# om-ai-lab/OmChat

Hardware: AMD Instinct MI355X
Metric: images/sec prefill + decode tokens/sec, OmChat-13B TP=1/8; p50 TTFT (higher is better)
Workload: dtype bf16

## Files before the change

### include/omchat_hip.h

```cpp
#ifndef OMCHAT_HIP_H
#define OMCHAT_HIP_H
#include <stddef.h>
#include <stdint.h>

#ifdef __cplusplus
extern "C" {
#endif

#define OMCHAT_F16 0
#define OMCHAT_BF16 1
#define OMCHAT_F32 2
#define OMCHAT_PAD_ROW INT32_MIN

typedef struct omchat_ctx omchat_ctx;

typedef struct {
  int v_hidden;
  int v_heads;
  int v_qk_channels;
  int v_mlp;
  int v_layers;
  int v_patch;
  int v_image;
  float v_eps;
// ... 53 lines not shown
                        const int32_t* seen_ids, const int32_t* n_seen_per_row, void* stream);
int omchat_set_sampling_filters(omchat_ctx* ctx, double min_p, double typical_p, double epsilon_cutoff, double eta_cutoff, void* stream);
int omchat_sample(omchat_ctx* ctx, const float* logits, int b, int32_t* next_tokens, void* stream);
#define OMCHAT_CON_MAX_NGRAM 64
#define OMCHAT_CON_MAX_EOS 16
#define OMCHAT_CON_MAX_SUPPRESS 1024
#define OMCHAT_CON_MAX_BAD_WORDS 1024
#define OMCHAT_CON_MAX_BAD_WORD_IDS 8192
int omchat_set_constraints(omchat_ctx* ctx, int b, int no_repeat_ngram_size, int min_new_tokens, int min_length, const int32_t* eos_ids, int n_eos,
                           const int32_t* suppress_ids, int n_suppress, const int32_t* begin_suppress_ids, int n_begin_suppress,
                           const int32_t* bad_word_ids, const int32_t* bad_word_offsets, int n_bad_words, const int32_t* prompt_ids,
                           const int32_t* prompt_len, int max_new, void* stream);
#define OMCHAT_FSM_MAX_STATES (1 << 20)
#define OMCHAT_FSM_MAX_EDGES (1 << 26)
#define OMCHAT_FSM_DEAD (-1)
int omchat_fsm_load(omchat_ctx* ctx, int n_states, const int32_t* off, const int32_t* tok, const int32_t* nxt, void* stream);
int omchat_fsm_begin(omchat_ctx* ctx, int b, const int32_t* start_states, int max_new, void* stream);
int omchat_fsm_states(omchat_ctx* ctx, int b, int32_t* out, void* stream);
int omchat_set_logprobs(omchat_ctx* ctx, int b, int max_new, void* stream);
int omchat_read_logprobs(omchat_ctx* ctx, int b, float* raw, float* processed, int32_t* counts, int max_len);
#define OMCHAT_LP_MAX_TOP 20
#define OMCHAT_LP_MAX_SCORED 32
int omchat_set_logprobs_ex(omchat_ctx* ctx, int b, int max_new, int top_n, const int32_t* score_ids, int n_score, void* stream);
int omchat_read_logprob_extras(omchat_ctx* ctx, int b, float* top_vals, int32_t* top_ids, float* scored, int32_t* counts, int max_len);
int omchat_read_sampling_state(omchat_ctx* ctx, int row, int* step, uint32_t* seen_words);
int omchat_kv_lengths(omchat_ctx* ctx, int32_t* out, int b);
int omchat_kv_rewind(omchat_ctx* ctx, int b, int n, void* stream);

int omchat_beam_begin(omchat_ctx* ctx, int b, int num_beams, float length_penalty, int early_stopping, const int32_t* eos_ids, int n_eos,
                      int max_new, int prompt_tok_len, void* stream);
int omchat_beam_step(omchat_ctx* ctx, const float* logits, int rows, int32_t* next_tokens, int32_t* done_word, void* stream);
int omchat_beam_result(omchat_ctx* ctx, int num_return, int32_t* tokens, int32_t* lengths, float* scores, int max_len);

int omchat_group_begin(omchat_ctx* ctx, int b, int N, int prompt_len, int share, void* stream);
int omchat_group_share_available(omchat_ctx* ctx, int N);

#define OMCHAT_VERIFY_KEEP_ALL 1
#define OMCHAT_VERIFY_SAMPLE 2
int omchat_decode_verify(omchat_ctx* ctx, const int32_t* tokens, int T, float* logits, int32_t* picks,
                         int* n_accept, int flags, void* stream);

int omchat_prefill_extend(omchat_ctx* ctx, const void* embeds, int S_new, int keep, float* logits_last, void* hidden_out, void* stream);
int omchat_extend_attn_form(int S_new, int keep, int Hkv);
int omchat_kv_read(omchat_ctx* ctx, int layer, int which, int pos0, int n, void* out, void* stream);
int omchat_kv_read_row(omchat_ctx* ctx, int row, int layer, int which, int pos0, int n, void* out, void* stream);

int omchat_prefill_suffixes(omchat_ctx* ctx, const void* embeds, int N, int S_max, const int32_t* lengths, int keep, float* logits_last,
                            void* hidden_out, void* stream);
int omchat_suffix_attn_form(int shared, int n_rep);

int omchat_enable_decode_graph(omchat_ctx* ctx, int on);
int omchat_decode_graph_stats(omchat_ctx* ctx, long* steps, long* replays, long* captures);
int omchat_bf16x12_stats(omchat_ctx* ctx, int* roles, long* launches, int* coded);

int omchat_enable_fp8_decode(omchat_ctx* ctx, int on);

int omchat_enable_mxfp4_decode(omchat_ctx* ctx, int mode);

enum omchat_weight_format {
  OMCHAT_WFMT_16 = 0,
  OMCHAT_WFMT_16_PACKED = 1,
  OMCHAT_WFMT_E4M3 = 2,
  OMCHAT_WFMT_MXFP4 = 3,
  OMCHAT_WFMT_MXFP4_PACKED = 4,
  OMCHAT_WFMT_COUNT = 5
};
int omchat_decode_weight_format(int rows, int fp8_on, int mxfp4_mode, int packed16_ready, int geometry_ok, int* x_pack_nb);

int omchat_enable_fp8_kv(omchat_ctx* ctx, int on);
int omchat_enable_fp8_prefill(omchat_ctx* ctx, int on);

#define OMCHAT_PROF_DECODE_GATEUP 0
#define OMCHAT_PROF_PREFILL_GATEUP 1
#define OMCHAT_PROF_VIT_FC1 2
#define OMCHAT_PROF_CATS 3
int omchat_prof_enable(omchat_ctx* ctx, int on);
int omchat_prof_read(omchat_ctx* ctx, int cat, double* total_ms, long* launches, int reset);

int omchat_mha_fwd(const void* qkv, int B, int S, int H, float softmax_scale, int causal, void* out, int dtype, void* stream);
int omchat_mha_fwd_varlen(const void* qkv, int B, int S, int H, int D, const int32_t* seqlens, float softmax_scale, int causal,
                          void* out, int dtype, void* stream);

int omchat_op_gemm(int dtype, const void* A, int lda, const void* W, int ldw, void* C, int ldc, int M, int N, int K,
                   const void* bias, const void* ls, const void* resid, int ldr, int epi, int force_tile, void* stream);
int omchat_op_gemm_fused(int dtype, const void* A, int lda, const void* W, int ldw, void* C, int ldc, int M, int N, int K,
                         const void* bias, const void* ls, const void* resid, int ldr, int epi, int force_tile, const float* row_scale,
                         const float* rs_stats, int rs_ld, int rs_nslots, int rs_dim, float rs_eps,
                         float* stats, int stats_ld, int* nslots, void* stream);
int omchat_op_stats_finish(const float* stats, int ld, int slot0, int nslots, int ngroups, int rows, int dim, float eps, float* out, void* stream);
int omchat_op_row_sumsq(int dtype, const void* x, int ldx, int rows, int H, float* stats, void* stream);
int omchat_op_fold_cols(int dtype, const void* W, const void* n, void* out, int rows, int cols, void* stream);
int omchat_op_vit_knorm_slots(int dtype, void* k, int ld, const void* wk, int rows, int C, int C_total, float eps, const float* stats, int stats_ld,
                              int nslots, float* sumsq_q, void* stream);
int omchat_op_mha_qnorm(int dtype, const void* qkv, int B, int Sq, int H, const float* sumsq, int stride, int dim, const void* wq,
                        float eps, float q_scale, void* out, void* stream);
int omchat_op_gemv_norm(int dtype, const void* X, const void* W, int ldw, void* Y, int N, int K, const void* norm_w, float eps,
                        const void* bias, int epi, int out_f32, void* stream);
int omchat_op_set_tuning(int key, int value);
int omchat_gemm_tune_load(const char* path);
int omchat_gemm_tune_dump(const char* path);
long omchat_gemm_tune_runs(void);
size_t omchat_op_gemm_sk_ws(void);
int omchat_op_gemm_sk(int dtype, const void* A, int lda, const void* W, int ldw, void* C, int ldc, int M, int N, int K,
                      const void* bias, const void* ls, const void* resid, int ldr, int epi, int force_tile, void* ws,
                      size_t ws_bytes, int stream_k, void* stream);
int omchat_op_gemv(int dtype, const void* X, int ldx, const void* W, int ldw, void* Y, int ldy, int b, int N, int K,
                   const void* bias, const void* resid, int ldr, int epi, int out_f32, void* stream);
int omchat_op_gemv_packed(int dtype, const void* X, int ldx, const void* W, int ldw, void* Y, int ldy, int b, int N, int K,
                          const void* bias, int epi, int out_f32, int ksplit, int w_packed, int y_packed, void* stream);
int omchat_op_pack_x(int dtype, const void* X, int ldx, int b, int K, void* out, void* stream);
int omchat_op_gemm_fp8(int dtype, const void* A8, const float* a_scale, const void* W8, const float* w_scale, void* C, int ldc, int M, int N,
                       int K, const void* bias, const void* resid, int ldr, int epi, void* stream);
int omchat_op_quant_rows_fp8(int dtype, const void* x, const void* norm_w, float eps, void* y8, float* scale, int rows, int H, void* stream);
int omchat_op_quant_fp8(int dtype, const void* W, int N, int K, void* W8, float* scale, void* stream);
int omchat_op_gemv_fp8(int dtype, const void* X, const void* W8, const float* scale, void* Y, int N, int K, const void* bias,
                       const void* resid, int epi, int out_f32, int ksplit, void* stream);
int omchat_op_quant_mxfp4(int dtype, const void* W, int N, int K, void* W4, void* S, void* stream);
int omchat_op_gemv_mxfp4(int dtype, const void* X, const void* W4, const void* S, void* Y, int N, int K, const void* bias,
                         const void* resid, int epi, int out_f32, int ksplit, void* stream);
int omchat_op_gemv_mxfp4_norm(int dtype, const void* X, const void* W4, const void* S, void* Y, int N, int K, const void* norm_w, float eps,
                              const void* bias, int epi, int out_f32, void* stream);
int omchat_op_gemv_mxfp4_rows(int dtype, const void* X, int ldx, const void* W4, const void* S, void* Y, int ldy, int b, int N, int K,
                              const void* bias, int epi, int out_f32, int ksplit, void* stream);
int omchat_op_gemv_mxfp4_packed(int dtype, const void* X, int ldx, const void* W4, const void* S, void* Y, int ldy, int b, int N, int K,
                                const void* bias, int epi, int out_f32, int ksplit, int y_packed, void* stream);
int omchat_op_encode_bf16x12(const void* W, int N, int K, void* coded, void* top, void* cnt, void* patch, void* over, void* stream);
int omchat_op_gemv_bf16x12(const void* X, const void* coded, const void* top, const void* cnt, const void* patch, void* Y, int N, int K,
                           const void* norm_w, float eps, const void* resid, int epi, int out_f32, void* stream);
int omchat_op_pack_w(int dtype, const void* W, int ldw, int N, int K, void* out, void* stream);
int omchat_op_pack_w4(const void* W4, const void* S, int N, int K, void* W4P, void* SP, void* stream);
int omchat_op_gemv_prepacked(int dtype, const void* XP, const void* WP, const void* SP, void* Y, int ldy, int b, int N, int K, const void* bias,
                             int epi, int out_f32, int ksplit, int y_packed, void* stream);
int omchat_op_rmsnorm(int dtype, const void* x, const void* w, void* y, int rows, int H, float eps, void* stream);
int omchat_op_resid_rmsnorm(int dtype, void* x, int ldx, const float* part, int ks, const void* w, void* xn, int ldn, int rows, int H,
                            float eps, int pack_nb, void* stream);
int omchat_op_vit_qknorm(int dtype, void* qkv, int ld, const void* wq, const void* wk, int rows, int C, int C_total,
                         float eps, float q_scale, void* stream);
int omchat_op_attn_prefill(int dtype, const void* q, const void* k, const void* v, void* out, int b, int Sq, int Skv,
                           int Hq, int Hkv, const int32_t* kv_len, int causal, int q_pos0, float scale, void* stream);
int omchat_op_attn_prefill_d(int dtype, const void* q, const void* k, const void* v, void* out, int b, int Sq, int Skv,
                             int Hq, int Hkv, int D, const int32_t* kv_len, int causal, int q_pos0, float scale, void* stream);
int omchat_op_layernorm(int dtype, const void* x, const void* w, const void* b, void* y, int rows, int H, float eps, void* stream);
size_t omchat_op_attn_decode_ws(int b, int Hq, int L);
int omchat_op_attn_decode(int dtype, const void* q, const void* k, const void* v, void* out, int b, int Hq, int Hkv,
                          int cap, int L, const int32_t* kv_len, float scale, void* ws, size_t ws_bytes, void* stream);
int omchat_op_attn_verify(int dtype, const void* q, void* k, void* v, void* out, int T, int Hq, int Hkv, int cap, int L, float scale,
                          void* ws, size_t ws_bytes, void* stream);
int omchat_op_attn_verify_tpw(int keys, int Hkv);
size_t omchat_op_attn_extend_ws(int Sq, int Hq, int Hkv, int L);
int omchat_op_attn_extend(int dtype, const void* q, const void* k, const void* v, void* out, int Sq, int Hq, int Hkv, int cap, int L,
                          float scale, void* ws, size_t ws_bytes, void* stream);
size_t omchat_op_attn_shared_ws(int G, int N, int Hq, int Hkv, int P, int L);
int omchat_op_attn_shared(int dtype, const void* q, void* k, void* v, void* out, int G, int N, int Hq, int Hkv, int cap, int P, int L,
                          float scale, void* ws, size_t ws_bytes, void* stream);
int omchat_op_attn_shared_lens(int dtype, const void* q, void* k, void* v, void* out, int G, int N, int Hq, int Hkv, int cap, int P, int L,
                               const int* kv_len, float scale, void* ws, size_t ws_bytes, void* stream);
size_t omchat_op_attn_suffix_ws(int N, int S, int Hq, int Hkv, int P);
int omchat_op_attn_suffix(int dtype, const void* q, const void* k, const void* v, void* out, int N, int S, int Hq, int Hkv, int cap, int P,
                          const int32_t* lengths, int* kv_len_dev, float scale, void* ws, size_t ws_bytes, void* stream);
int omchat_op_attn_verify_append(int dtype, const void* qkv, float theta, void* k, void* v, void* out, int T, int Hq, int Hkv, int cap,
                                 int L, float scale, void* ws, size_t ws_bytes, void* stream);
int omchat_op_attn_decode_kv8(int dtype, const void* q, const void* k8, const void* v8, const float* ks, const float* vs, void* out, int b,
                              int Hq, int Hkv, int cap, int L, const int32_t* kv_len, float scale, void* ws, size_t ws_bytes, void* stream);
int omchat_op_attn_decode_kv8_append(int dtype, void* qkv, float theta, void* k8, void* v8, float* ks, float* vs, void* k16, void* v16, void* out,
                                     int b, int Hq, int Hkv, int cap, int L, const int32_t* kv_len, const int32_t* pos, float scale, void* ws,
                                     size_t ws_bytes, void* stream);
int omchat_op_rope_kv(int dtype, void* qkv, int b, int S, int Hq, int Hkv, int pos0, float theta, void* kcache, void* vcache,
                      int cap, void* stream);
int omchat_op_rope_kv_q8(int dtype, void* qkv, int b, int S, int Hq, int Hkv, int pos0, float theta, void* kcache, void* vcache, int cap,
                         void* k8, void* v8, float* ks, float* vs, void* stream);
int omchat_op_argmax(const float* logits, int b, int V, int32_t* out, void* stream);
int omchat_op_attn_prefill_left(int dtype, const void* q, const void* k, const void* v, void* out, int b, int Sq, int Skv, int Hq, int Hkv,
                                const int32_t* kv_len, const int32_t* kv_start, int causal, int q_pos0, float scale, int fill_uniform, void* stream);
int omchat_op_rope_kv_pos(int dtype, void* qkv, int b, int S, int Hq, int Hkv, const int32_t* pos, int pos0, int slot0, int max_pos, float theta,
                          void* kcache, void* vcache, int cap, void* stream);
int omchat_op_argmax_ld(const float* logits, int ld, int b, int V, int32_t* out, int32_t* adv_pos, int32_t* adv_len, void* stream);
int omchat_op_im2col(int dtype, const void* pixels, void* cols, int B, int HW, int patch, int Kpad, void* stream);
int omchat_op_vit_assemble(int dtype, const void* pe, const void* cls, const void* pos, void* x, int B, int np, int C, void* stream);
int omchat_op_gather_rows(int dtype, const int32_t* idx, const void* table, const void* feats, void* out, int rows, int H, void* stream);
int omchat_op_copy_rows(int dtype, const void* src, int64_t src_ld, void* dst, int64_t dst_ld, int rows, int H, int group, int skip, void* stream);
int omchat_op_tp_finish(int dtype, const float* sum, const void* bias, const void* ls, const void* resid, void* out, int M, int N, int epi, void* stream);
// ... 82 lines not shown
```

### omchat_amd/_lib.py

```python
import ctypes as C
import os

HERE = os.path.dirname(os.path.abspath(__file__))
LIB_PATH = os.environ.get("OMCHAT_LIB") or os.path.join(HERE, "lib", "libomchat_hip.so")
_lib = None

F16, BF16, F32 = 0, 1, 2
EPI_NONE, EPI_GELU, EPI_LS_RESID, EPI_RESID, EPI_SWIGLU = 0, 1, 2, 3, 4
EPI_F32OUT = 6
EPI_LS_RESID_STATS, EPI_NONE_STATS = 7, 8
PAD_ROW = -(2 ** 31)
PROF_DECODE_GATEUP, PROF_PREFILL_GATEUP, PROF_VIT_FC1 = 0, 1, 2


class OmchatConfig(C.Structure):
    _fields_ = [
        ("v_hidden", C.c_int), ("v_heads", C.c_int), ("v_qk_channels", C.c_int), ("v_mlp", C.c_int), ("v_layers", C.c_int),
        ("v_patch", C.c_int), ("v_image", C.c_int), ("v_eps", C.c_float),
        ("t_hidden", C.c_int), ("t_layers", C.c_int), ("t_heads", C.c_int), ("t_kv_heads", C.c_int), ("t_mlp", C.c_int),
        ("t_vocab", C.c_int), ("t_vocab_total", C.c_int), ("t_eps", C.c_float), ("rope_theta", C.c_float),
        ("max_seq", C.c_int), ("max_batch", C.c_int), ("max_tiles", C.c_int), ("max_prefill_rows", C.c_int), ("dtype", C.c_int),
        ("v_head_dim", C.c_int), ("v_norm_type", C.c_int), ("v_no_qk_norm", C.c_int),
    ]

# ... 43 lines not shown
    "omchat_beam_step": (_i, [_vp, _vp, _i, _vp, _vp, _vp]),
    "omchat_beam_result": (_i, [_vp, _i, _vp, _vp, _vp, _i]),
    "omchat_decode_verify": (_i, [_vp, _vp, _i, _vp, _vp, _vp, _i, _vp]),
    "omchat_decode_step_masked": (_i, [_vp, _vp, _i, _vp, _vp, _i, _vp, _vp, _vp]),
    "omchat_masked_decode_begin": (_i, [_vp, _i, _vp, _vp, _i, _i, _vp]),
    "omchat_decode_step_masked_next": (_i, [_vp, _vp, _i, _vp, _vp, _vp]),
    "omchat_fused_status": (_i, [_vp, C.POINTER(C.c_long), C.POINTER(C.c_uint)]),
    "omchat_has_experiments": (_i, []),
    "omchat_set_allreduce_hook": (_i, [_vp, _vp, _vp]),
    "omchat_allreduce_noop": (_i, [_vp, _vp, C.c_size_t, _i, _vp]),
    "omchat_op_gemv_norm": (_i, [_i, _vp, _vp, _i, _vp, _i, _i, _vp, _f, _vp, _i, _i, _vp]),
    "omchat_prof_enable": (_i, [_vp, _i]),
    "omchat_prof_read": (_i, [_vp, _i, C.POINTER(C.c_double), C.POINTER(C.c_long), _i]),
    "omchat_mha_fwd": (_i, [_vp, _i, _i, _i, _f, _i, _vp, _i, _vp]),
    "omchat_mha_fwd_varlen": (_i, [_vp, _i, _i, _i, _i, _vp, _f, _i, _vp, _i, _vp]),
    "omchat_op_gemm": (_i, [_i, _vp, _i, _vp, _i, _vp, _i, _i, _i, _i, _vp, _vp, _vp, _i, _i, _i, _vp]),
    "omchat_op_gemm_fused": (_i, [_i, _vp, _i, _vp, _i, _vp, _i, _i, _i, _i, _vp, _vp, _vp, _i, _i, _i, _vp, _vp, _i, _i, _i, _f, _vp, _i, _vp, _vp]),
    "omchat_op_stats_finish": (_i, [_vp, _i, _i, _i, _i, _i, _i, _f, _vp, _vp]),
    "omchat_op_row_sumsq": (_i, [_i, _vp, _i, _i, _i, _vp, _vp]),
    "omchat_op_fold_cols": (_i, [_i, _vp, _vp, _vp, _i, _i, _vp]),
    "omchat_op_vit_knorm_slots": (_i, [_i, _vp, _i, _vp, _i, _i, _i, _f, _vp, _i, _i, _vp, _vp]),
    "omchat_op_mha_qnorm": (_i, [_i, _vp, _i, _i, _i, _vp, _i, _i, _vp, _f, _f, _vp, _vp]),
    "omchat_ctx_sp_stats": (_i, [_vp, C.POINTER(C.c_long), C.POINTER(C.c_long)]),
    "omchat_op_set_tuning": (_i, [_i, _i]),
    "omchat_gemm_tune_load": (_i, [C.c_char_p]),
    "omchat_gemm_tune_dump": (_i, [C.c_char_p]),
    "omchat_gemm_tune_runs": (C.c_long, []),
    "omchat_op_gemm_sk_ws": (_sz, []),
    "omchat_op_gemm_sk": (_i, [_i, _vp, _i, _vp, _i, _vp, _i, _i, _i, _i, _vp, _vp, _vp, _i, _i, _i, _vp, _sz, _i, _vp]),
    "omchat_op_gemv": (_i, [_i, _vp, _i, _vp, _i, _vp, _i, _i, _i, _i, _vp, _vp, _i, _i, _i, _vp]),
    "omchat_op_gemv_packed": (_i, [_i, _vp, _i, _vp, _i, _vp, _i, _i, _i, _i, _vp, _i, _i, _i, _i, _i, _vp]),
    "omchat_op_pack_x": (_i, [_i, _vp, _i, _i, _i, _vp, _vp]),
    "omchat_op_gemm_fp8": (_i, [_i, _vp, _vp, _vp, _vp, _vp, _i, _i, _i, _i, _vp, _vp, _i, _i, _vp]),
    "omchat_op_quant_rows_fp8": (_i, [_i, _vp, _vp, _f, _vp, _vp, _i, _i, _vp]),
    "omchat_enable_fp8_decode": (_i, [_vp, _i]),
    "omchat_enable_fp8_kv": (_i, [_vp, _i]),
    "omchat_enable_fp8_prefill": (_i, [_vp, _i]),
    "omchat_enable_decode_graph": (_i, [_vp, _i]),
    "omchat_bf16x12_stats": (_i, [_vp, C.POINTER(_i), C.POINTER(C.c_long), C.POINTER(_i)]),
    "omchat_decode_graph_stats": (_i, [_vp, C.POINTER(C.c_long), C.POINTER(C.c_long), C.POINTER(C.c_long)]),
    "omchat_op_quant_fp8": (_i, [_i, _vp, _i, _i, _vp, _vp, _vp]),
    "omchat_op_gemv_fp8": (_i, [_i, _vp, _vp, _vp, _vp, _i, _i, _vp, _vp, _i, _i, _i, _vp]),
    "omchat_enable_mxfp4_decode": (_i, [_vp, _i]),
    "omchat_decode_weight_format": (_i, [_i, _i, _i, _i, _i, C.POINTER(_i)]),
    "omchat_op_quant_mxfp4": (_i, [_i, _vp, _i, _i, _vp, _vp, _vp]),
    "omchat_op_gemv_mxfp4": (_i, [_i, _vp, _vp, _vp, _vp, _i, _i, _vp, _vp, _i, _i, _i, _vp]),
    "omchat_op_gemv_mxfp4_rows": (_i, [_i, _vp, _i, _vp, _vp, _vp, _i, _i, _i, _i, _vp, _i, _i, _i, _vp]),
    "omchat_op_gemv_mxfp4_packed": (_i, [_i, _vp, _i, _vp, _vp, _vp, _i, _i, _i, _i, _vp, _i, _i, _i, _i, _vp]),
    "omchat_op_pack_w": (_i, [_i, _vp, _i, _i, _i, _vp, _vp]),
    "omchat_op_pack_w4": (_i, [_vp, _vp, _i, _i, _vp, _vp, _vp]),
    "omchat_op_gemv_prepacked": (_i, [_i, _vp, _vp, _vp, _vp, _i, _i, _i, _i, _vp, _i, _i, _i, _i, _vp]),
    "omchat_op_encode_bf16x12": (_i, [_vp, _i, _i, _vp, _vp, _vp, _vp, _vp, _vp]),
    "omchat_op_gemv_bf16x12": (_i, [_vp, _vp, _vp, _vp, _vp, _vp, _i, _i, _vp, _f, _vp, _i, _i, _vp]),
    "omchat_op_gemv_mxfp4_norm": (_i, [_i, _vp, _vp, _vp, _vp, _i, _i, _vp, _f, _vp, _i, _i, _vp]),
    "omchat_op_rmsnorm": (_i, [_i, _vp, _vp, _vp, _i, _i, _f, _vp]),
    "omchat_op_resid_rmsnorm": (_i, [_i, _vp, _i, _vp, _i, _vp, _vp, _i, _i, _i, _f, _i, _vp]),
    "omchat_op_vit_qknorm": (_i, [_i, _vp, _i, _vp, _vp, _i, _i, _i, _f, _f, _vp]),
    "omchat_op_attn_prefill": (_i, [_i, _vp, _vp, _vp, _vp, _i, _i, _i, _i, _i, _vp, _i, _i, _f, _vp]),
    "omchat_op_attn_prefill_d": (_i, [_i, _vp, _vp, _vp, _vp, _i, _i, _i, _i, _i, _i, _vp, _i, _i, _f, _vp]),
    "omchat_op_layernorm": (_i, [_i, _vp, _vp, _vp, _vp, _i, _i, _f, _vp]),
    "omchat_op_attn_decode_ws": (_sz, [_i, _i, _i]),
    "omchat_op_attn_decode": (_i, [_i, _vp, _vp, _vp, _vp, _i, _i, _i, _i, _i, _vp, _f, _vp, _sz, _vp]),
    "omchat_op_attn_verify_tpw": (_i, [_i, _i]),
    "omchat_op_attn_verify": (_i, [_i, _vp, _vp, _vp, _vp, _i, _i, _i, _i, _i, _f, _vp, _sz, _vp]),
    "omchat_op_attn_extend_ws": (_sz, [_i, _i, _i, _i]),
    "omchat_op_attn_shared_ws": (_sz, [_i, _i, _i, _i, _i, _i]),
    "omchat_op_attn_shared": (_i, [_i, _vp, _vp, _vp, _vp, _i, _i, _i, _i, _i, _i, _i, _f, _vp, _sz, _vp]),
    "omchat_op_attn_extend": (_i, [_i, _vp, _vp, _vp, _vp, _i, _i, _i, _i, _i, _f, _vp, _sz, _vp]),
    "omchat_prefill_extend": (_i, [_vp, _vp, _i, _i, _vp, _vp, _vp]),
    "omchat_extend_attn_form": (_i, [_i, _i, _i]),
    "omchat_kv_read": (_i, [_vp, _i, _i, _i, _i, _vp, _vp]),
    "omchat_kv_read_row": (_i, [_vp, _i, _i, _i, _i, _i, _vp, _vp]),
    "omchat_prefill_suffixes": (_i, [_vp, _vp, _i, _i, _vp, _i, _vp, _vp, _vp]),
    "omchat_suffix_attn_form": (_i, [_i, _i]),
    "omchat_op_attn_shared_lens": (_i, [_i, _vp, _vp, _vp, _vp, _i, _i, _i, _i, _i, _i, _i, _vp, _f, _vp, _sz, _vp]),
    "omchat_op_attn_suffix_ws": (_sz, [_i, _i, _i, _i, _i]),
    "omchat_op_attn_suffix": (_i, [_i, _vp, _vp, _vp, _vp, _i, _i, _i, _i, _i, _i, _vp, _vp, _f, _vp, _sz, _vp]),
    "omchat_op_attn_verify_append": (_i, [_i, _vp, _f, _vp, _vp, _vp, _i, _i, _i, _i, _i, _f, _vp, _sz, _vp]),
    "omchat_op_attn_decode_kv8": (_i, [_i, _vp, _vp, _vp, _vp, _vp, _vp, _i, _i, _i, _i, _i, _vp, _f, _vp, _sz, _vp]),
    "omchat_op_attn_decode_kv8_append": (_i, [_i, _vp, _f, _vp, _vp, _vp, _vp, _vp, _vp, _vp, _i, _i, _i, _i, _i, _vp, _vp, _f, _vp, _sz, _vp]),
    "omchat_op_rope_kv": (_i, [_i, _vp, _i, _i, _i, _i, _i, _f, _vp, _vp, _i, _vp]),
    "omchat_op_rope_kv_q8": (_i, [_i, _vp, _i, _i, _i, _i, _i, _f, _vp, _vp, _i, _vp, _vp, _vp, _vp, _vp]),
    "omchat_op_argmax": (_i, [_vp, _i, _i, _vp, _vp]),
    "omchat_op_attn_prefill_left": (_i, [_i, _vp, _vp, _vp, _vp, _i, _i, _i, _i, _i, _vp, _vp, _i, _i, _f, _i, _vp]),
    "omchat_op_rope_kv_pos": (_i, [_i, _vp, _i, _i, _i, _i, _vp, _i, _i, _i, _f, _vp, _vp, _i, _vp]),
    "omchat_op_argmax_ld": (_i, [_vp, _i, _i, _i, _vp, _vp, _vp, _vp]),
    "omchat_op_im2col": (_i, [_i, _vp, _vp, _i, _i, _i, _i, _vp]),
    "omchat_op_vit_assemble": (_i, [_i, _vp, _vp, _vp, _vp, _i, _i, _i, _vp]),
    "omchat_op_gather_rows": (_i, [_i, _vp, _vp, _vp, _vp, _i, _i, _vp]),
    "omchat_op_copy_rows": (_i, [_i, _vp, _i64, _vp, _i64, _i, _i, _i, _i, _vp]),
    "omchat_op_tp_finish": (_i, [_i, _vp, _vp, _vp, _vp, _vp, _i, _i, _i, _vp]),
    "omchat_op_resid16_norm": (_i, [_i, _vp, _i, _vp, _i, _vp, _vp, _vp, _i, _i, _i, _f, _vp]),
    "omchat_op_cast_f32": (_i, [_i, _vp, _vp, _i64, _vp]),
    "omchat_op_rmsnorm_ld": (_i, [_i, _vp, _i, _vp, _vp, _i, _i, _i, _f, _i, _vp]),
    "omchat_op_layernorm_ld": (_i, [_i, _vp, _i, _vp, _vp, _vp, _i, _i, _i, _f, _vp]),
    "omchat_op_sample": (_i, [_vp, _i, _i, _u64, _f, _i, C.c_double, _f, _vp, _vp, _i, _vp, _vp, _vp]),
    "omchat_op_token_logprob": (_i, [_vp, _i, _i, _i, _vp, _vp, _f, _f, _vp, _vp, _vp, _vp, _vp, _vp, _vp]),
    "omchat_op_lse_label_ws": (_sz, [_i, _i]),
    "omchat_op_lse_label": (_i, [_i, _vp, _i, _vp, _i, _i, _i, _i, _vp, _vp, _vp, _vp, _sz, _vp]),
    "omchat_op_top_logprobs": (_i, [_vp, _i, _i, _i, _i, _vp, _i, _vp, _vp, _vp, _vp]),
    "omchat_op_sample_filtered": (_i, [_vp, _i, _i, _u64, _f, _i, C.c_double, _f, C.c_double, C.c_double, C.c_double, C.c_double, _vp, _vp, _i,
                                       _vp, _vp, _vp, _vp]),
    "omchat_op_sample_verify": (_i, [_vp, _i, _i, _i, _vp, _u64, _i, _f, _i, C.c_double, _f, C.c_double, C.c_double, C.c_double, C.c_double, _vp,
                                     _i, _i, _i, _vp, _vp, _vp, _vp]),
    "omchat_read_sampling_state": (_i, [_vp, _i, _vp, _vp]),
    "omchat_op_token_logprob_interval": (_i, [_vp, _i, _i, _i, _vp, _vp, _f, _f, _vp, _vp, _vp, _vp, _vp, _vp, _vp, _vp]),
# ... 83 lines not shown
```

### omchat_amd/csrc/capi.hip

```cpp
#include "kernels.h"
#include <stdlib.h>
#include "../../include/omchat_hip.h"
#include <math.h>
#include <vector>

#define S(x) ((hipStream_t)(x))
#if OMCHAT_EXPERIMENTS
int g_launch_any_order = 0;
#endif

extern "C" int omchat_op_gemm(int dtype, const void* A, int lda, const void* W, int ldw, void* C, int ldc, int M, int N, int K,
                              const void* bias, const void* ls, const void* resid, int ldr, int epi, int force_tile, void* stream) {
  GemmArgs g{A, lda, W, ldw, C, ldc, M, N, K, bias, ls, resid, ldr, epi, force_tile, nullptr, 0, -1};
  return launch_gemm(dtype, g, S(stream));
}

extern "C" int omchat_op_gemm_fused(int dtype, const void* A, int lda, const void* W, int ldw, void* C, int ldc, int M, int N, int K,
                                    const void* bias, const void* ls, const void* resid, int ldr, int epi, int force_tile, const float* row_scale,
                                    const float* rs_stats, int rs_ld, int rs_nslots, int rs_dim, float rs_eps,
                                    float* stats, int stats_ld, int* nslots, void* stream) {
  GemmArgs g{A, lda, W, ldw, C, ldc, M, N, K, bias, ls, resid, ldr, epi, force_tile, nullptr, 0, -1};
  g.row_scale = row_scale; g.stats = stats; g.stats_ld = stats_ld; g.stats_nslots = nslots;
  g.rs_stats = rs_stats; g.rs_ld = rs_ld; g.rs_nslots = rs_nslots; g.rs_dim = rs_dim; g.rs_eps = rs_eps;
  return launch_gemm(dtype, g, S(stream));
// ... 20 lines not shown
  a.K = (const char*)qkv + (size_t)H * 128 * 2; a.k_sb = a.q_sb; a.k_sh = 128; a.k_sr = row;
  a.V = (const char*)qkv + (size_t)2 * H * 128 * 2; a.v_sb = a.q_sb; a.v_sh = 128; a.v_sr = row;
  a.O = out; a.o_sb = (int64_t)Sq * H * 128; a.o_sh = 128; a.o_sr = (int64_t)H * 128;
  a.batch = B; a.q_heads = H; a.kv_heads = H; a.Sq = Sq; a.Skv = Sq; a.kv_len = nullptr; a.causal = 0; a.q_pos0 = 0;
  a.scale = 1.0f;
  a.qn_sumsq = sumsq; a.qn_stride = stride; a.qn_dim = dim; a.qn_w = wq; a.qn_eps = eps; a.qn_scale = q_scale;
  return launch_attn_prefill(dtype, a, S(stream));
}

extern "C" int omchat_op_set_tuning(int key, int value) {
  const char* allow = getenv("OMCHAT_ALLOW_TUNING");
  if (!allow || allow[0] != '1') {
    omchat_set_error("omchat_op_set_tuning: process-global test / measurement hook; set OMCHAT_ALLOW_TUNING=1 to use it (see include/omchat_hip.h)");
    return 1;
  }
  if (key == 0) { gemm_set_skew(value); return 0; }
  if (key == 1) { gemv_set_force_mfma(value); return 0; }
  if (key == 5) { gemm_set_autotune(value); return 0; }
  if (key == 4) { model_set_ar_min_rows(value); return 0; }
  if (key == 6) { model_set_pack_replica(value); return 0; }
  if (key == 8) { attn_set_v2(value); return 0; }
  if (key == 9) { model_set_fuse_peer_norm(value); return 0; }
  if (key == 10) { attn_set_tpw(value); return 0; }
  if (key == 11) { gemv_set_no_xs(value); return 0; }
  if (key == 12) { attn_set_klds(value); return 0; }
  if (key == 25) { attn_set_dma(value); return 0; }
  if (key == 26) { attn_set_dma_slots(value); return 0; }
  if (key == 27) { attn_set_dma_rot(value); return 0; }
  if (key == 28) { gemv_set_skew(value); return 0; }
  if (key == 29) { model_set_tp_f32(value); return 0; }
  if (key == 30) { attn_set_hsplit(value); return 0; }
  if (key == 33) { attn_set_mha_xcd(value); return 0; }
  if (key == 16) { gemv_set_norm_loop(value); return 0; }
  if (key == 17) { gemv_set_rows_balance(value); return 0; }
  if (key == 19) { attn_set_merge_mid_min(value); return 0; }
  if (key == 21) { attn_set_merge_dg(value); return 0; }
  if (key == 13) { gemm_set_persist(value); return 0; }
  if (key == 14) { model_set_norm_in_gemv(value); return 0; }
  if (key == 22) { model_set_fuse_attn_oproj(value); return 0; }
  if (key == 23) { model_set_decode_layer(value); return 0; }
  if (key == 24) { gemv_set_dyn(value); return 0; }
  if (key == 34) { gemv_set_shard_shapes(value); return 0; }
  if (key == 35) { model_set_shard_as_tp1(value); return 0; }
  if (key == 36) { attn_set_kg(value); return 0; }
  if (key == 37) { gemm_set_wide_store(value); return 0; }
  if (key == 43) { gemm_set_skip_dead(value); return 0; }
  if (key == 44) { model_set_vit_fused(value); return 0; }
  if (key == 45) { model_set_tp_sp(value); return 0; }
  if (key == 46) { attn_set_peel(value); return 0; }
  if (key == 47) { attn_set_kv8_tpw(value); return 0; }
  if (key == 48) { attn_set_kv8_fuse(value); return 0; }
  if (key == 49) { model_set_extend_attn(value); return 0; }
  if (key == 50) { model_set_x12_roles(value); return 0; }
  if (key == 51) { model_set_suffix_attn(value); return 0; }
  if (key == 38) { gemv_set_gu_rr(value); return 0; }
  if (key == 39) { gemv_set_longk_direct(value); return 0; }
  if (key == 40) { norm_set_wave(value); return 0; }
#if OMCHAT_EXPERIMENTS
  if (key == 41) { g_launch_any_order = value; return 0; }
  if (key == 42) { model_set_ao_oproj(value); return 0; }
#endif
  omchat_set_error("omchat_op_set_tuning: unknown key");
  return 1;
}

extern "C" int omchat_allreduce_noop(void*, void*, size_t, int, void*) { return 0; }

extern "C" int omchat_gemm_tune_load(const char* path) { OM_CHECK(path, "null path"); return gemm_tune_load(path); }
extern "C" int omchat_gemm_tune_dump(const char* path) { OM_CHECK(path, "null path"); return gemm_tune_dump(path); }
extern "C" long omchat_gemm_tune_runs(void) { return gemm_tune_runs(); }

extern "C" size_t omchat_op_gemm_sk_ws(void) { return gemm_sk_ws_bytes(); }

extern "C" int omchat_op_gemm_sk(int dtype, const void* A, int lda, const void* W, int ldw, void* C, int ldc, int M, int N, int K,
                                 const void* bias, const void* ls, const void* resid, int ldr, int epi, int force_tile, void* ws,
                                 size_t ws_bytes, int stream_k, void* stream) {
  GemmArgs g{A, lda, W, ldw, C, ldc, M, N, K, bias, ls, resid, ldr, epi, force_tile, ws, ws_bytes, stream_k};
  return launch_gemm(dtype, g, S(stream));
}

extern "C" int omchat_op_gemv(int dtype, const void* X, int ldx, const void* W, int ldw, void* Y, int ldy, int b, int N, int K,
                              const void* bias, const void* resid, int ldr, int epi, int out_f32, void* stream) {
  GemvArgs g{X, ldx, W, ldw, Y, ldy, b, N, K, bias, resid, ldr, epi, out_f32};
  return launch_gemv(dtype, g, S(stream));
}

extern "C" int omchat_op_gemv_norm(int dtype, const void* X, const void* W, int ldw, void* Y, int N, int K, const void* norm_w, float eps,
                                   const void* bias, int epi, int out_f32, void* stream) {
  OM_CHECK(X && W && Y && norm_w, "null argument");
  GemvArgs g{X, K, W, ldw, Y, N, 1, N, K, bias, nullptr, 0, epi, out_f32};
  g.norm_w = norm_w; g.norm_eps = eps;
  return launch_gemv(dtype, g, S(stream));
}

extern "C" int omchat_op_gemv_packed(int dtype, const void* X, int ldx, const void* W, int ldw, void* Y, int ldy, int b, int N, int K,
                                     const void* bias, int epi, int out_f32, int ksplit, int w_packed, int y_packed, void* stream) {
  OM_CHECK(b >= 1 && b <= 32 && K % 64 == 0, "1 <= b <= 32, K % 64 == 0");
  const int NB = b > 16 ? 2 : 1;
  void *xp = nullptr, *wp = nullptr;
  OM_HIP(hipMalloc(&xp, (size_t)NB * 16 * K * 2));
  int rc = launch_pack_x(dtype, X, ldx, b, K, xp, S(stream));
  if (rc == 0 && w_packed) {
    if (hipMalloc(&wp, (size_t)N * K * 2) != hipSuccess) { hipFree(xp); omchat_set_error("hipMalloc failed"); return 2; }
    rc = launch_pack_w(dtype, W, ldw, N, K, wp, S(stream));
  }
  if (rc == 0) {
// ... 698 lines not shown
  const int NB = b > 16 ? 2 : 1;
  void *xp = nullptr, *wp = nullptr, *sp = nullptr;
  auto drop = [&]() { if (xp) hipFree(xp); if (wp) hipFree(wp); if (sp) hipFree(sp); };
  if (hipMalloc(&xp, (size_t)NB * 16 * K * 2) != hipSuccess || hipMalloc(&wp, (size_t)N * (K / 2)) != hipSuccess ||
      hipMalloc(&sp, (size_t)N * (K / 32)) != hipSuccess) {
    (void)hipGetLastError(); drop(); omchat_set_error("hipMalloc failed"); return 2;
  }
  int rc = launch_pack_x(dtype, X, ldx, b, K, xp, S(stream));
  if (rc == 0) rc = launch_pack_w4(W4, (const unsigned char*)S_, N, K, wp, (unsigned char*)sp, S(stream));
  if (rc == 0) {
    GemvArgs g{xp, K, wp, K / 2, Y, ldy, b, N, K, bias, nullptr, 0, epi, out_f32, ksplit, 0, nullptr, 1, 1, y_packed};
    g.mx_scale = (const unsigned char*)sp;
    rc = launch_gemv(dtype, g, S(stream));
  }
  hipStreamSynchronize(S(stream));
  drop();
  return rc;
}

extern "C" int omchat_op_pack_w(int dtype, const void* W, int ldw, int N, int K, void* out, void* stream) { return launch_pack_w(dtype, W, ldw, N, K, out, S(stream)); }
extern "C" int omchat_op_pack_w4(const void* W4, const void* S_, int N, int K, void* W4P, void* SP, void* stream) {
  return launch_pack_w4(W4, (const unsigned char*)S_, N, K, W4P, (unsigned char*)SP, S(stream));
}
extern "C" int omchat_op_gemv_prepacked(int dtype, const void* XP, const void* WP, const void* SP, void* Y, int ldy, int b, int N, int K, const void* bias,
                                        int epi, int out_f32, int ksplit, int y_packed, void* stream) {
  OM_CHECK(XP && WP && Y, "null argument");
  OM_CHECK(b >= 1 && b <= 32 && K >= 64 && K % 64 == 0 && N >= 16 && N % 16 == 0, "pre-packed GEMV: 1 <= b <= 32, K % 64 == 0, N % 16 == 0");
  GemvArgs g{XP, K, WP, SP ? K / 2 : K, Y, ldy, b, N, K, bias, nullptr, 0, epi, out_f32, ksplit, 0, nullptr, 1, 1, y_packed};
  g.mx_scale = (const unsigned char*)SP;
  return launch_gemv(dtype, g, S(stream));
}

extern "C" int omchat_op_gemv_mxfp4_norm(int dtype, const void* X, const void* W4, const void* S_, void* Y, int N, int K, const void* norm_w,
                                         float eps, const void* bias, int epi, int out_f32, void* stream) {
  OM_CHECK(X && W4 && S_ && Y && norm_w, "null argument");
  OM_CHECK(K % 32 == 0, "MXFP4: K must be a multiple of 32 (one e8m0 scale per 32 consecutive k)");
  GemvArgs g{X, K, W4, K / 2, Y, N, 1, N, K, bias, nullptr, 0, epi, out_f32};
  g.norm_w = norm_w; g.norm_eps = eps;
  g.mx_scale = (const unsigned char*)S_;
  return launch_gemv(dtype, g, S(stream));
}

extern "C" int omchat_op_encode_bf16x12(const void* W, int N, int K, void* coded, void* top, void* cnt, void* patch, void* over, void* stream) {
  return launch_encode_bf16x12(W, K, N, K, coded, (unsigned char*)top, (unsigned char*)cnt, (unsigned*)patch, (int*)over, S(stream));
}
extern "C" int omchat_op_gemv_bf16x12(const void* X, const void* coded, const void* top, const void* cnt, const void* patch, void* Y, int N, int K,
                                      const void* norm_w, float eps, const void* resid, int epi, int out_f32, void* stream) {
  OM_CHECK(X && coded && top && cnt && patch && Y, "null argument");
  GemvArgs g{X, K, coded, K / 2 * 3, Y, N, 1, N, K, nullptr, resid, N, epi, out_f32};
  g.norm_w = norm_w; g.norm_eps = eps;
  g.x12_top = (const unsigned char*)top; g.x12_cnt = (const unsigned char*)cnt; g.x12_patch = (const unsigned*)patch;
  return launch_gemv(OMCHAT_BF16, g, S(stream));
}

extern "C" int omchat_op_attn_prefill_d(int dtype, const void* q, const void* k, const void* v, void* out, int b, int Sq, int Skv, int Hq,
                                        int Hkv, int D, const int32_t* kv_len, int causal, int q_pos0, float scale, void* stream) {
  AttnArgs a{};
  a.Q = q; a.q_sb = (int64_t)Sq * Hq * D; a.q_sh = D; a.q_sr = (int64_t)Hq * D;
  a.K = k; a.k_sb = (int64_t)Hkv * Skv * D; a.k_sh = (int64_t)Skv * D; a.k_sr = D;
  a.V = v; a.v_sb = a.k_sb; a.v_sh = a.k_sh; a.v_sr = D;
  a.O = out; a.o_sb = a.q_sb; a.o_sh = D; a.o_sr = a.q_sr;
  a.batch = b; a.q_heads = Hq; a.kv_heads = Hkv; a.Sq = Sq; a.Skv = Skv; a.kv_len = kv_len; a.causal = causal; a.q_pos0 = q_pos0; a.scale = scale;
  a.head_dim = D;
  return launch_attn_prefill(dtype, a, S(stream));
}

extern "C" int omchat_op_layernorm(int dtype, const void* x, const void* w, const void* b, void* y, int rows, int H, float eps, void* stream) {
  return launch_layernorm(dtype, x, H, w, b, y, H, rows, H, eps, S(stream));
}

extern "C" int omchat_op_attn_prefill_left(int dtype, const void* q, const void* k, const void* v, void* out, int b, int Sq, int Skv, int Hq,
                                           int Hkv, const int32_t* kv_len, const int32_t* kv_start, int causal, int q_pos0, float scale,
                                           int fill_uniform, void* stream) {
  OM_CHECK(q && k && v && out && kv_start, "null argument");
  AttnArgs a{};
  a.Q = q; a.q_sb = (int64_t)Sq * Hq * 128; a.q_sh = 128; a.q_sr = (int64_t)Hq * 128;
  a.K = k; a.k_sb = (int64_t)Hkv * Skv * 128; a.k_sh = (int64_t)Skv * 128; a.k_sr = 128;
  a.V = v; a.v_sb = a.k_sb; a.v_sh = a.k_sh; a.v_sr = 128;
  a.O = out; a.o_sb = a.q_sb; a.o_sh = 128; a.o_sr = a.q_sr;
  a.batch = b; a.q_heads = Hq; a.kv_heads = Hkv; a.Sq = Sq; a.Skv = Skv; a.kv_len = kv_len; a.kv_start = kv_start; a.causal = causal;
  a.q_pos0 = q_pos0; a.scale = scale;
  int rc = launch_attn_prefill(dtype, a, S(stream));
  if (!rc && fill_uniform) rc = launch_attn_uniform_rows(dtype, a, S(stream));
  return rc;
}

extern "C" int omchat_op_rope_kv_pos(int dtype, void* qkv, int b, int Sq, int Hq, int Hkv, const int32_t* pos, int pos0, int slot0, int max_pos,
                                     float theta, void* kcache, void* vcache, int cap, void* stream) {
  OM_CHECK(qkv && kcache && vcache && b >= 1 && Sq >= 1 && Hq >= 1 && Hkv >= 1 && max_pos >= 1 && cap >= 1 && slot0 >= -1, "bad argument");
  if (pos) {
    std::vector<int32_t> hp((size_t)b * Sq);
    OM_HIP(hipStreamSynchronize(S(stream)));
    OM_HIP(hipMemcpy(hp.data(), pos, hp.size() * 4, hipMemcpyDeviceToHost));
    for (int32_t p : hp) {
      OM_CHECK(p >= 0 && p < max_pos, "position outside the RoPE table");
      OM_CHECK(slot0 >= 0 || p < cap, "cache slot exceeds the capacity");
    }
  } else {
    OM_CHECK(pos0 >= 0 && pos0 + Sq <= max_pos, "position outside the RoPE table");
    OM_CHECK(slot0 >= 0 || pos0 + Sq <= cap, "cache slot exceeds the capacity");
  }
  OM_CHECK(slot0 < 0 || slot0 + Sq <= cap, "cache slot exceeds the capacity");
  float* d = rope_table_device(max_pos, theta);
  OM_CHECK(d, "rope table allocation failed");
  RopeArgs r{qkv, (Hq + 2 * Hkv) * 128, b * Sq, Sq, Hq, Hkv, pos, pos0, d, max_pos, kcache, vcache, (int64_t)Hkv * cap * 128, (int64_t)cap * 128};
  r.slot0 = slot0;
// ... 57 lines not shown
```

### omchat_amd/csrc/ctx.h

```cpp
#pragma once
#include "kernels.h"
#include "../../include/omchat_hip.h"
#include <rccl/rccl.h>
#include <string>
#include <unordered_map>
#include <vector>

#define TRY(x) do { int rc_ = (x); if (rc_) return rc_; } while (0)

extern int g_fuse_peer_norm;

enum RouteKind { R_PLAIN = 0, R_GATE = 1, R_UP = 2, R_PATCH = 3 };
struct Route {
  void* dst = nullptr;
  int64_t rows = 0, cols = 0;
  int64_t dst_ld = 0;
  int kind = R_PLAIN;
  bool loaded = false;
  float synth_std = 0.02f, synth_off = 0.f;
};

struct Grown {
  void* p = nullptr; size_t cap = 0;
  void release() { if (p) (void)hipFree(p); p = nullptr; cap = 0; }
// ... 54 lines not shown
  int fsm_cap = 0, fsm_fed = 0;
  int *fsm_cnt = nullptr;
  int32_t* fsm_cur = nullptr;
  uint32_t* fsm_bm = nullptr; int fsm_bmw = 0;
  bool sampling_on() const { return smp.on; }
  bool constraints_on() const { return con.on; }
  bool logprobs_on() const { return lp.on; }
  bool fsm_on() const { return fsm.on; }
  void release() { con_hist.release(); lp_rec.release(); lp_xrec.release(); fsm_mem.release(); fsm_trail.release(); }
};

struct BeamState {
  struct Search { bool on = false; int b = 0, N = 0, KB = 0, max_new = 0, P = 0, es = 0, ns = 1, t = 0; float lp = 1.f; std::vector<int> eos; };
  Search cur;
  Grown state, table, dn, parents, stash;
  bool stash8 = false;
  std::vector<int> hpos, hlen;
  bool on() const { return cur.on; }
  void end() { cur.on = false; }
  void release() { for (Grown* g : {&state, &table, &dn, &parents, &stash}) g->release(); }
};

struct GroupState {
  bool share = false; int b = 0, N = 0, P = 0;
  Grown ws;
  std::vector<int> hpos, hlen;
  bool on() const { return share; }
  void end() { share = false; }
  void release() { ws.release(); }
};

struct omchat_ctx {
  omchat_config c;
  int dt = OMCHAT_BF16;
  int tp_rank = 0, tp_size = 1;
  ncclComm_t comm = nullptr;
  std::vector<void*> allocs;
  size_t bytes = 0;
  std::unordered_map<std::string, Route> routes;

  int v_np = 0, v_ntok = 0, v_Cq = 0, v_kpad = 0, v_hd = 128;
  int t_qdim = 0, t_kvdim = 0, t_qkvdim = 0;

  struct VitLayer { void *ls1, *ls2, *n1, *n2, *n1b, *n2b, *wqkv, *qn, *kn, *wproj, *bproj, *w1, *b1, *w2, *b2; };
  struct DecLayer { void *ln1, *ln2, *wqkv, *bqkv, *wo, *wgu, *wd; };
  enum Proj { P_QKV = 0, P_O = 1, P_GU = 2, P_DOWN = 3, P_LM = 4 };
  struct WRef { void* W = nullptr; int ldw = 0; float* w_scale = nullptr; unsigned char* mx_scale = nullptr; int packed = 0; };
  enum WState { W_ABSENT = 0, W_BUILT, W_STALE, W_UNAVAILABLE };
  struct WTable { std::vector<WRef> e; int state = W_ABSENT; };
  WTable wt[OMCHAT_WFMT_COUNT];
  const WRef* layer_w(int fmt, int layer) const { return &wt[fmt].e[(size_t)layer * 4]; }
  const WRef& lm_w(int fmt) const { return wt[fmt].e.back(); }
  bool built(int fmt) const { return wt[fmt].state == W_BUILT; }
  enum X12Role { X12_GU = 0, X12_DOWN = 1, X12_LM = 2, X12_ROLES = 3 };
  struct X12Ref { void* W = nullptr; unsigned char* top = nullptr; unsigned char* cnt = nullptr; unsigned* patch = nullptr; bool ok = false; };
  struct X12Table { std::vector<X12Ref> e; int state = W_ABSENT; };
  X12Table x12[X12_ROLES];
  int* x12_over = nullptr;
  long x12_launches[X12_ROLES] = {0, 0, 0};
  bool fp8_decode = false;
  int mxfp4_mode = 0;
  void *k8cache = nullptr, *v8cache = nullptr;
  float *ks8 = nullptr, *vs8 = nullptr;
  bool fp8_kv = false, kv8_valid = false, fp8_prefill = false;
  void* tw_q8 = nullptr; float* tw_q8s = nullptr;
  int64_t scale_layer_stride() const { return (int64_t)c.max_batch * c.t_kv_heads * c.max_seq; }
  struct DecodeGraph { hipGraph_t graph = nullptr; hipGraphExec_t exec = nullptr; int cap_len = 0, grp_N = 0, grp_P = 0; const void* grp_ws = nullptr; };
  std::unordered_map<int, DecodeGraph> graphs;
  bool graph_on = false;
  hipStream_t graph_stream = nullptr;
  hipEvent_t graph_ev_in = nullptr, graph_ev_out = nullptr;
  int32_t *d_tok_in = nullptr, *d_tok_out = nullptr;
  long graph_steps = 0, graph_replays = 0, graph_captures = 0;
  void *v_cls = nullptr, *v_pos = nullptr, *v_wpatch = nullptr, *v_bpatch = nullptr;
  std::vector<VitLayer> vl;
  void *p_w0 = nullptr, *p_b0 = nullptr, *p_w2 = nullptr, *p_b2 = nullptr;
  void *t_embed = nullptr, *t_norm = nullptr, *t_lm = nullptr;
  std::vector<DecLayer> dl;
  float* rope = nullptr;

  void *vw_cols = nullptr, *vw_pe = nullptr, *vw_x = nullptr, *vw_x2 = nullptr, *vw_xn = nullptr, *vw_qkv = nullptr, *vw_ao = nullptr,
       *vw_h = nullptr, *vw_feat = nullptr, *vw_proj = nullptr;
  float* vw_sumsq = nullptr;
  float *vw_stats_x = nullptr, *vw_stats_qk = nullptr, *vw_rstd = nullptr;
  int vw_stats_x_ld = 0, vw_stats_qk_ld = 0, vw_stats_x_ld_used = 1;
  struct VitFold { void *wqkv = nullptr, *w1 = nullptr; };
  std::vector<VitFold> vfold;
  bool vfold_stale = true;
  void *tw_x = nullptr, *tw_x2 = nullptr, *tw_xn = nullptr, *tw_qkv = nullptr, *tw_ao = nullptr, *tw_act = nullptr, *tw_last = nullptr;
  float* tw_logits = nullptr;
  void* sk_ws = nullptr; size_t sk_ws_bytes = 0;
  float* tp_f32_ws = nullptr; size_t tp_f32_bytes = 0;
  float* tw_part = nullptr;
  float* tw_attn_ws = nullptr;
  size_t tw_attn_ws_bytes = 0;
  void* fd_ws = nullptr;
  unsigned* fd_err = nullptr;
  unsigned fd_epoch = 0;
  long n_fused_launches = 0;
  void* dl_ws = nullptr;
  long n_layer_launches = 0;
  unsigned long long* dbg_stamps = nullptr;
  unsigned* dyn_ctr = nullptr;
  int *d_pos = nullptr, *d_len = nullptr, *d_idx = nullptr, *d_start = nullptr;
  int* d_verify_n = nullptr;
  PickState pick;
  BeamState beam;
  GroupState group;
  Grown ext_ws;
  Grown score_ws;
  int grow(Grown& g, size_t n) {
    if (n <= g.cap) return 0;
// ... 168 lines not shown
```

### omchat_amd/csrc/gemv.hip

```cpp
#include "kernels.h"
#include "rowdot.h"
#include <type_traits>

namespace {

struct GemvP {
  const void* X; const void* W; void* Y; const void* bias; const void* resid;
  int ldx, ldw, ldy, ldr, b, N, K, out_f32, ksplit;
  const float* w_scale;
  int y_packed;
  const void* norm_w; float norm_eps;
  unsigned* dyn;
  void* y_pack;
  unsigned long long* dbg;
  const unsigned char* mx_s;
  const unsigned char* x12_top;
  const unsigned char* x12_cnt;
  const unsigned* x12_patch;
#if OMCHAT_EXPERIMENTS
  int xskew;
#endif
};
constexpr int WF_16 = 0, WF_E4M3 = 1, WF_MX4 = 2, WF_X12 = 3;
#if OMCHAT_EXPERIMENTS
// ... 653 lines not shown
  s.pv = p.x12_patch[row * 32 + (lane & 31)];
}
__device__ __forceinline__ void x12_row_finish(X12Row& s) {
  const int t = __builtin_amdgcn_readfirstlane((int)s.top_raw) - 7;
  s.cnt = __builtin_amdgcn_readfirstlane((int)s.cnt_raw);
  s.pi = 0;
  s.tlo = ((unsigned)((t + 1) & 0x7f) << 8) | ((unsigned)((t + 2) & 0x7f) << 16) | ((unsigned)((t + 3) & 0x7f) << 24);
  s.thi = (unsigned)((t + 4) & 0x7f) | ((unsigned)((t + 5) & 0x7f) << 8) | ((unsigned)((t + 6) & 0x7f) << 16) | ((unsigned)((t + 7) & 0x7f) << 24);
}
__device__ __forceinline__ rw_u32x4 x12_decode(const X12W& w, const X12Row& s) {
  const unsigned n = w.nib;
  const unsigned c0 = n & 0x07070707u, c1 = (n >> 4) & 0x07070707u;
  unsigned h0 = __builtin_amdgcn_perm(s.thi, s.tlo, c0), h1 = __builtin_amdgcn_perm(s.thi, s.tlo, c1);
  h0 |= (n & 0x08080808u) << 4;
  h1 |= n & 0x80808080u;
  rw_u32x4 r;
  r.x = __builtin_amdgcn_perm(h0, w.lo.x, 0x05010400u);
  r.y = __builtin_amdgcn_perm(h0, w.lo.x, 0x07030602u);
  r.z = __builtin_amdgcn_perm(h1, w.lo.y, 0x05010400u);
  r.w = __builtin_amdgcn_perm(h1, w.lo.y, 0x07030602u);
  return r;
}
__device__ __forceinline__ void x12_apply(rw_u32x4& w, unsigned e, int lane) {
  const unsigned k = e >> 16, i = k & 7u, sh = (i & 1u) * 16u;
  const unsigned keep = ~(0xffffu << sh), ins = (e & 0xffffu) << sh;
  const bool mine = lane == (int)((k >> 3) & 63u);
  w.x = (mine && (i >> 1) == 0u) ? ((w.x & keep) | ins) : w.x;
  w.y = (mine && (i >> 1) == 1u) ? ((w.y & keep) | ins) : w.y;
  w.z = (mine && (i >> 1) == 2u) ? ((w.z & keep) | ins) : w.z;
  w.w = (mine && (i >> 1) == 3u) ? ((w.w & keep) | ins) : w.w;
}
template <int G>
__device__ __forceinline__ void x12_group(rw_u32x4 (&wd)[G], const X12W* w, X12Row& s, int chunk0, int nch, int lane) {
#pragma unroll
  for (int i = 0; i < G; ++i) wd[i] = x12_decode(w[i], s);
  while (s.pi < s.cnt) {
    const unsigned e = (unsigned)__builtin_amdgcn_readlane((int)s.pv, s.pi);
    const int ch = (int)(e >> 25) - chunk0;
    if (ch >= G) break;
#pragma unroll
    for (int i = 0; i < G; ++i) if (ch == i) x12_apply(wd[i], e, lane);
    ++s.pi;
  }
  if (chunk0 + G > nch) {
    for (int j = 0; j < s.cnt; ++j) {
      const unsigned e = (unsigned)__builtin_amdgcn_readlane((int)s.pv, j);
      if ((e >> 19) != 0u) break;
#pragma unroll
      for (int i = 0; i < G; ++i) if (chunk0 + i >= nch) x12_apply(wd[i], e, 0);
    }
  }
}

template <typename T, int WF>
__device__ __forceinline__ typename RwW<WF>::type rw_ldw(const GemvP& p, size_t row, int k) {
  if constexpr (WF == WF_X12) return x12_ldw(p, row, k >> 9, (k >> 3) & 63); else
  if constexpr (WF == WF_E4M3) {
    return __builtin_nontemporal_load(reinterpret_cast<const rw_u32x2*>((const unsigned char*)p.W + row * p.ldw + k));
  } else if constexpr (WF == WF_MX4) {
    rw_u32x2 w;
    w.x = __builtin_nontemporal_load(reinterpret_cast<const unsigned*>((const unsigned char*)p.W + row * p.ldw + (k >> 1)));
    w.y = __builtin_nontemporal_load(p.mx_s + row * (size_t)(p.K >> 5) + (k >> 5));
    return w;
  } else {
    return __builtin_nontemporal_load(reinterpret_cast<const rw_u32x4*>((const T*)p.W + row * p.ldw + k));
  }
}
template <typename T, int WF>
__device__ __forceinline__ float rw_dotw(typename RwW<WF>::type w, rw_u32x4 x, float acc) {
  if constexpr (WF == WF_E4M3) return rw_dot8_fp8<T>(w, x, acc);
  else if constexpr (WF == WF_MX4) return fmaf(rw_dot8_fp4<T>(w.x, x), mx_scale_of(w.y), acc);
  else return rw_dot8<T>(w, x, acc);
}

template <typename T, int R> struct RwTail { const T* p0; const T* p1; int idx[R]; float v0[R], v1[R]; };
template <typename T, int R> __device__ __forceinline__ void rw_tail_load(RwTail<T, R>& t) {
#pragma unroll
  for (int r = 0; r < R; ++r) { t.v0[r] = tof(t.p0[t.idx[r]]); t.v1[r] = tof(t.p1[t.idx[r]]); }
}
template <typename T, int R, int NCH, int WF>
__device__ __forceinline__ void rw_rows_q(const GemvP& p, const int (&rows)[R], int k0, int lane, const rw_u32x4 (&xr)[RW_MAXC], float (&acc)[R],
                                          RwTail<T, R>& tail) {
  typename RwW<WF>::type w[R][NCH];
#pragma unroll
  for (int r = 0; r < R; ++r)
#pragma unroll
    for (int c = 0; c < NCH; ++c) {
      int k = k0 + c * 512 + lane * 8;
      k = k < p.K ? k : k0;
      w[r][c] = rw_ldw<T, WF>(p, (size_t)rows[r], k);
    }
  float sc[R];
#pragma unroll
  for (int r = 0; r < R; ++r) sc[r] = WF == WF_E4M3 ? p.w_scale[rows[r]] : 1.f;
  rw_tail_load<T, R>(tail);
#pragma unroll
  for (int r = 0; r < R; ++r) {
    float a = 0.f;
#pragma unroll
    for (int c = 0; c < NCH; ++c) a = rw_dotw<T, WF>(w[r][c], xr[c], a);
#pragma unroll
    for (int o = 32; o > 0; o >>= 1) a += __shfl_xor(a, o, 64);
    acc[r] = WF == WF_E4M3 ? a * sc[r] : a;
  }
}

template <typename T, int R, int N, int WF>
__device__ __forceinline__ void rw_dispatch_q(int nch, const GemvP& p, const int (&rows)[R], int k0, int lane, const rw_u32x4 (&xr)[RW_MAXC],
                                              float (&acc)[R], RwTail<T, R>& tail) {
  if constexpr (N > 0) {
    if (nch == N) rw_rows_q<T, R, N, WF>(p, rows, k0, lane, xr, acc, tail);
    else rw_dispatch_q<T, R, N - 1, WF>(nch, p, rows, k0, lane, xr, acc, tail);
  }
}

template <typename T, int R, int NCH>
__device__ __forceinline__ void rw_rows(const T* W, int ldw, const int (&rows)[R], int k0, int K, int lane, const rw_u32x4 (&xr)[RW_MAXC],
                                        float (&acc)[R], RwTail<T, R>& tail) {
  rw_u32x4 w[R][NCH];
#pragma unroll
  for (int r = 0; r < R; ++r)
#pragma unroll
    for (int c = 0; c < NCH; ++c) {
      int k = k0 + c * 512 + lane * 8;
      k = k < K ? k : k0;
      w[r][c] = __builtin_nontemporal_load(reinterpret_cast<const rw_u32x4*>(W + (size_t)rows[r] * ldw + k));
    }
  rw_tail_load<T, R>(tail);
#pragma unroll
  for (int r = 0; r < R; ++r) {
    float a = 0.f;
#pragma unroll
    for (int c = 0; c < NCH; ++c) a = rw_dot8<T>(w[r][c], xr[c], a);
#pragma unroll
    for (int o = 32; o > 0; o >>= 1) a += __shfl_xor(a, o, 64);
    acc[r] = a;
  }
}

template <typename T, int R, int N>
__device__ __forceinline__ void rw_dispatch(int nch, const T* W, int ldw, const int (&rows)[R], int k0, int K, int lane,
                                            const rw_u32x4 (&xr)[RW_MAXC], float (&acc)[R], RwTail<T, R>& tail) {
  if constexpr (N > 0) {
    if (nch == N) rw_rows<T, R, N>(W, ldw, rows, k0, K, lane, xr, acc, tail);
    else rw_dispatch<T, R, N - 1>(nch, W, ldw, rows, k0, K, lane, xr, acc, tail);
  }
}

template <typename T, int EPI, int RR, int WAVES, int F8>
__device__ __forceinline__ void gemv_rows_body(const GemvP& p) {
  constexpr int R = EPI == EPI_SWIGLU ? 2 * RR : RR;
  constexpr int OUT = RR;
  const int lane = threadIdx.x & 63, wave = threadIdx.x >> 6;
  const T* W = (const T*)p.W;
  if constexpr (EPI == EPI_RESID && WAVES == 7) OM_DBG_MIN(1, blockIdx.x < 8);
  const int nch_all = (p.K + 511) / 512;
  const int c_lo = (int)(((long)nch_all * blockIdx.y) / p.ksplit), c_hi = (int)(((long)nch_all * (blockIdx.y + 1)) / p.ksplit);
  const int nch = c_hi - c_lo, k0 = c_lo * 512;
  rw_u32x4 xr[RW_MAXC];
#pragma unroll
  for (int c = 0; c < RW_MAXC; ++c) {
    const int k = k0 + c * 512 + lane * 8;
    rw_u32x4 z = {0u, 0u, 0u, 0u};
    xr[c] = (c < nch && k < p.K) ? *reinterpret_cast<const rw_u32x4*>((const T*)p.X + k) : z;
  }
  const int n_out = EPI == EPI_SWIGLU ? p.N / 2 : p.N;
  const int ngroups = (n_out + OUT - 1) / OUT;
  for (int g = blockIdx.x * WAVES + wave; g < ngroups; g += gridDim.x * WAVES) {
    int rows[R];
#pragma unroll
    for (int r = 0; r < R; ++r) {
      if constexpr (EPI == EPI_SWIGLU) {
        int n = g * RR + (r % RR); n = n < n_out ? n : n_out - 1;
        rows[r] = 32 * (n >> 4) + (n & 15) + (r / RR) * 16;
      } else {
        const int n = g * R + r;
        rows[r] = n < p.N ? n : p.N - 1;
      }
    }
    float acc[R];
    RwTail<T, R> tail;
    {
      constexpr bool plain = EPI != EPI_SWIGLU && EPI != EPI_PARTIAL;
      const bool hb = plain && p.bias, hr = EPI == EPI_RESID && !p.out_f32;
      tail.p0 = hb ? (const T*)p.bias : (const T*)p.X;
      tail.p1 = hr ? (const T*)p.resid : (const T*)p.X;
#pragma unroll
      for (int r = 0; r < R; ++r) {
        const int n = g * OUT + r;
        tail.idx[r] = (hb || hr) ? (n < n_out ? n : n_out - 1) : 0;
      }
      if (!hb) tail.p0 = tail.p1;
      if (!hr) tail.p1 = tail.p0;
    }
    if constexpr (F8 != WF_16) rw_dispatch_q<T, R, RW_MAXC, F8>(nch, p, rows, k0, lane, xr, acc, tail);
    else rw_dispatch<T, R, RW_MAXC>(nch, W, p.ldw, rows, k0, p.K, lane, xr, acc, tail);
    if (lane == 0) {
#pragma unroll
      for (int r = 0; r < OUT; ++r) {
        const int n = g * OUT + r;
        if (n >= n_out) continue;
        if constexpr (EPI == EPI_SWIGLU) {
          const float gt = rnd<T>(acc[r]), up = rnd<T>(acc[r + RR]);
          ((T*)p.Y)[n] = fromf<T>(rnd<T>(silu(gt)) * up);
        } else if constexpr (EPI == EPI_PARTIAL) {
          ((float*)p.Y)[(size_t)blockIdx.y * p.ldy + n] = acc[r];
        } else {
          float y = acc[r] + (p.bias ? tail.v0[r] : 0.f);
          if (p.out_f32) ((float*)p.Y)[n] = y;
          else {
            y = rnd<T>(y);
            if constexpr (EPI == EPI_RESID) y = tail.v1[r] + y;
            ((T*)p.Y)[n] = fromf<T>(y);
          }
        }
      }
    }
  }
  if constexpr (EPI == EPI_RESID && WAVES == 7) OM_DBG_MAX(3, (blockIdx.x & 7) == 0);
}

template <typename T, int EPI, int RR = 4, int WAVES = 4, bool F8 = false>
__global__ __launch_bounds__(WAVES * 64) void gemv_rows_kernel(GemvP p) { gemv_rows_body<T, EPI, RR, WAVES, F8 ? WF_E4M3 : WF_16>(p); }
template <typename T, int EPI, int RR, int WAVES>
__global__ __launch_bounds__(WAVES * 64) void gemv_rows_mx4_kernel(GemvP p) { gemv_rows_body<T, EPI, RR, WAVES, WF_MX4>(p); }

template <typename T, int EPI, int RR, int NCH, int F8, int WAVES>
__device__ __forceinline__ void gemv_rows_norm_body(const GemvP& p) {
  typedef typename V8<T>::type v8;
  constexpr int R = EPI == EPI_SWIGLU ? 2 * RR : RR;
  __shared__ __attribute__((aligned(16))) T xs[NCH * 512];
  __shared__ float red[WAVES];
  const int lane = threadIdx.x & 63, wave = __builtin_amdgcn_readfirstlane(threadIdx.x >> 6);
  const int n_out = EPI == EPI_SWIGLU ? p.N / 2 : p.N;
  int g = blockIdx.x * WAVES + wave;
#if OMCHAT_EXPERIMENTS
  if constexpr (EPI == EPI_SWIGLU && RR == 1 && WAVES == 4) {
    if (p.xskew) {
      const int x = blockIdx.x & 7, j = blockIdx.x >> 3;
      const int base = ((n_out + 3) / 4) / 8;
      const int n_x = base + ((x & 1) ? -p.xskew : p.xskew);
      if (j >= n_x) return;
      g = (x * base + ((x & 1) ? p.xskew : 0) + j) * 4 + wave;
    }
  }
#endif
  if constexpr (EPI == EPI_SWIGLU) OM_DBG_MIN(4, blockIdx.x < 8);
  if constexpr (EPI == EPI_NONE) OM_DBG_MIN(8, blockIdx.x < 8);
  static_assert(WAVES >= 4 && NCH <= 8, "sum-of-squares order: four owner waves, up to two chunks each");
  constexpr int MC = (NCH + WAVES - 1) / WAVES;
  constexpr int SC = (NCH + 3) / 4;
  rw_u32x4 xq[MC], nq[MC], sq[SC];
#pragma unroll
  for (int i = 0; i < MC; ++i) {
    const int c = wave + WAVES * i, k = c * 512 + lane * 8;
    const rw_u32x4 z = {0u, 0u, 0u, 0u};
    const bool ok = c < NCH && k < p.K;
    xq[i] = ok ? *reinterpret_cast<const rw_u32x4*>((const T*)p.X + k) : z;
    nq[i] = ok ? *reinterpret_cast<const rw_u32x4*>((const T*)p.norm_w + k) : z;
  }
#pragma unroll
  for (int i = 0; i < SC; ++i) {
    if constexpr (WAVES == 4) {
      sq[i] = xq[i];
    } else {
      const int c = wave + 4 * i, k = c * 512 + lane * 8;
      const rw_u32x4 z = {0u, 0u, 0u, 0u};
      sq[i] = (wave < 4 && c < NCH && k < p.K) ? *reinterpret_cast<const rw_u32x4*>((const T*)p.X + k) : z;
    }
  }
  int rows[R];
#pragma unroll
  for (int r = 0; r < R; ++r) {
    if constexpr (EPI == EPI_SWIGLU) {
      int n = g * RR + (r % RR); n = n < n_out ? n : n_out - 1;
      rows[r] = 32 * (n >> 4) + (n & 15) + (r / RR) * 16;
    } else {
      const int n = g * R + r;
      rows[r] = n < p.N ? n : p.N - 1;
    }
  }
  typedef typename RwW<F8>::type wreg_t;
  wreg_t w[R][NCH];
#pragma unroll
  for (int r = 0; r < R; ++r)
#pragma unroll
    for (int c = 0; c < NCH; ++c) {
      int k = c * 512 + lane * 8;
      k = k < p.K ? k : 0;
      if constexpr (F8 == WF_X12) w[r][c] = x12_ldw(p, (size_t)rows[r], c, lane);
      else w[r][c] = rw_ldw<T, F8>(p, (size_t)rows[r], k);
    }
  float e_bias[RR], e_scale[R];
  {
    const T* bp = (EPI != EPI_SWIGLU && p.bias) ? (const T*)p.bias : (const T*)p.norm_w;
    const int nmax = (EPI != EPI_SWIGLU && p.bias) ? n_out - 1 : 0;
#pragma unroll
    for (int r = 0; r < RR; ++r) {
      const int n = g * RR + r;
      e_bias[r] = tof(bp[n < nmax ? n : nmax]);
    }
    if (!(EPI != EPI_SWIGLU && p.bias)) {
#pragma unroll
      for (int r = 0; r < RR; ++r) e_bias[r] = 0.f;
    }
#pragma unroll
    for (int r = 0; r < R; ++r) e_scale[r] = 1.f;
    if constexpr (F8 == WF_E4M3) {
#pragma unroll
      for (int r = 0; r < R; ++r) e_scale[r] = p.w_scale[rows[r]];
    }
  }
  X12Row xst[F8 == WF_X12 ? R : 1];
  if constexpr (F8 == WF_X12) {
#pragma unroll
    for (int r = 0; r < R; ++r) x12_row_load(xst[r], p, (size_t)rows[r], lane);
  }
  __builtin_amdgcn_sched_barrier(0);
  float ss = 0.f;
#pragma unroll
  for (int i = 0; i < SC; ++i) {
    const v8 xv = __builtin_bit_cast(v8, sq[i]);
#pragma unroll
    for (int j = 0; j < 8; ++j) { const float v = tof(xv[j]); ss += v * v; }
  }
#pragma unroll
  for (int o = 32; o > 0; o >>= 1) ss += __shfl_xor(ss, o, 64);
  if (lane == 0 && wave < 4) red[wave] = ss;
  asm volatile("s_waitcnt lgkmcnt(0)" ::: "memory");
  __builtin_amdgcn_s_barrier();
  float tot = red[0];
#pragma unroll
  for (int w = 1; w < 4; ++w) tot += red[w];
  const float inv = rsqrtf(tot / (float)p.K + p.norm_eps);
#pragma unroll
  for (int i = 0; i < MC; ++i) {
    const int c = wave + WAVES * i;
    if (c < NCH) {
      const v8 xv = __builtin_bit_cast(v8, xq[i]), wv = __builtin_bit_cast(v8, nq[i]);
      v8 o;
#pragma unroll
      for (int j = 0; j < 8; ++j) o[j] = fromf<T>(tof(wv[j]) * rnd<T>(tof(xv[j]) * inv));
      *reinterpret_cast<v8*>(xs + c * 512 + lane * 8) = o;
    }
  }
  asm volatile("s_waitcnt lgkmcnt(0)" ::: "memory");
  __builtin_amdgcn_s_barrier();
  rw_u32x4 xr[NCH];
#pragma unroll
  for (int c = 0; c < NCH; ++c) xr[c] = *reinterpret_cast<const rw_u32x4*>(xs + c * 512 + lane * 8);
  __builtin_amdgcn_sched_barrier(0);
  float acc[R];
#pragma unroll
  for (int r = 0; r < R; ++r) {
    float a = 0.f;
    if constexpr (F8 == WF_X12) x12_row_finish(xst[r]);
#pragma unroll
    for (int c = 0; c < NCH; ++c) {
      if constexpr (F8 != WF_X12) a = rw_dotw<T, F8>(w[r][c], xr[c], a);
    }
    if constexpr (F8 == WF_X12) {
      constexpr int G0 = NCH < 4 ? NCH : 4, G1 = NCH - G0;
      {
        rw_u32x4 wd[G0];
        x12_group<G0>(wd, &w[r][0], xst[r], 0, NCH, lane);
#pragma unroll
        for (int c = 0; c < G0; ++c) a = rw_dot8<T>(wd[c], xr[c], a);
      }
      if constexpr (G1 > 0) {
        rw_u32x4 wd[G1];
        x12_group<G1>(wd, &w[r][G0], xst[r], G0, NCH, lane);
#pragma unroll
        for (int c = 0; c < G1; ++c) a = rw_dot8<T>(wd[c], xr[G0 + c], a);
      }
    }
#pragma unroll
    for (int o = 32; o > 0; o >>= 1) a += __shfl_xor(a, o, 64);
    if constexpr (F8 == WF_E4M3) a *= e_scale[r];
    acc[r] = a;
  }
  if (lane == 0) {
#pragma unroll
    for (int r = 0; r < RR; ++r) {
      const int n = g * RR + r;
      if (n >= n_out) continue;
      if constexpr (EPI == EPI_SWIGLU) {
        const float gt = rnd<T>(acc[r]), up = rnd<T>(acc[r + RR]);
        ((T*)p.Y)[n] = fromf<T>(rnd<T>(silu(gt)) * up);
      } else {
        const float y = acc[r] + e_bias[r];
        if (p.out_f32) ((float*)p.Y)[n] = y;
        else ((T*)p.Y)[n] = fromf<T>(y);
      }
    }
  }
  if constexpr (EPI == EPI_SWIGLU) { OM_DBG_MAX(5, blockIdx.x + 64 >= gridDim.x); OM_DBG_MAX(16 + (blockIdx.x & 7), blockIdx.x + 512 >= gridDim.x); }
  if constexpr (EPI == EPI_NONE) OM_DBG_MAX(9, (blockIdx.x & 7) == 0);
}

template <typename T, int EPI, int RR, int NCH, bool F8, int WAVES = 4>
__global__ __launch_bounds__(WAVES * 64) void gemv_rows_norm_kernel(GemvP p) { gemv_rows_norm_body<T, EPI, RR, NCH, F8 ? WF_E4M3 : WF_16, WAVES>(p); }
template <typename T, int EPI, int RR, int NCH, int WAVES = 4>
__global__ __launch_bounds__(WAVES * 64) void gemv_rows_norm_mx4_kernel(GemvP p) { gemv_rows_norm_body<T, EPI, RR, NCH, WF_MX4, WAVES>(p); }
template <typename T, int EPI, int RR, int NCH>
__global__ __launch_bounds__(256) void gemv_rows_norm_x12_kernel(GemvP p) { gemv_rows_norm_body<T, EPI, RR, NCH, WF_X12, 4>(p); }

template <typename T, int EPI, int NCH, int F8>
__device__ __forceinline__ void gemv_rows_norm_loop_body(const GemvP& p, int per_wg, unsigned skew) {
  typedef typename V8<T>::type v8;
  constexpr int R = EPI == EPI_SWIGLU ? 2 : 1;
  __shared__ __attribute__((aligned(16))) T xs[NCH * 512];
  __shared__ float red[4];
  const int lane = threadIdx.x & 63, wave = __builtin_amdgcn_readfirstlane(threadIdx.x >> 6);
  const int n_out = EPI == EPI_SWIGLU ? p.N / 2 : p.N;
  int o0 = blockIdx.x * per_wg, o1 = o0 + per_wg < n_out ? o0 + per_wg : n_out;
  if constexpr (EPI == EPI_SWIGLU) OM_DBG_MIN(4, blockIdx.x < 8);
  if (skew) {
    const int l = blockIdx.x & 7;
    int pre = 0;
    for (int i = 0; i < l; ++i) pre += per_wg + (int)((skew >> (4 * i)) & 15u) - 8;
    o0 = (blockIdx.x >> 3) * 8 * per_wg + pre;
    o1 = o0 + per_wg + (int)((skew >> (4 * l)) & 15u) - 8;
    o1 = o1 < n_out ? o1 : n_out;
  }
  typedef typename RwW<F8>::type wreg_t;
  auto row_of = [&](int n, int r) { return EPI == EPI_SWIGLU ? 32 * (n >> 4) + (n & 15) + r * 16 : n; };
  auto load_w = [&](wreg_t (&w)[R][NCH], int n) {
#pragma unroll
    for (int r = 0; r < R; ++r) {
      const size_t row = (size_t)row_of(n, r);
#pragma unroll
      for (int c = 0; c < NCH; ++c) {
        int k = c * 512 + lane * 8;
        k = k < p.K ? k : 0;
        w[r][c] = rw_ldw<T, F8>(p, row, k);
      }
    }
  };
  wreg_t wa[R][NCH], wb[R][NCH], wc[R][NCH];
  const int u0 = o0 + wave;
  if (u0 < o1) load_w(wa, u0);
  if (u0 + 4 < o1) load_w(wb, u0 + 4);
  if (u0 + 8 < o1) load_w(wc, u0 + 8);
  constexpr int MC = (NCH + 3) / 4;
  rw_u32x4 xq[MC], nq[MC];
#pragma unroll
  for (int i = 0; i < MC; ++i) {
    const int c = wave + 4 * i, k = c * 512 + lane * 8;
    const rw_u32x4 z = {0u, 0u, 0u, 0u};
    const bool ok = c < NCH && k < p.K;
    xq[i] = ok ? *reinterpret_cast<const rw_u32x4*>((const T*)p.X + k) : z;
    nq[i] = ok ? *reinterpret_cast<const rw_u32x4*>((const T*)p.norm_w + k) : z;
  }
  __builtin_amdgcn_sched_barrier(0);
  float ss = 0.f;
#pragma unroll
  for (int i = 0; i < MC; ++i) {
    const v8 xv = __builtin_bit_cast(v8, xq[i]);
// ... 462 lines not shown
      if constexpr (F8 == WF_MX4) hipLaunchKernelGGL((gemv_rows_norm_mx4_kernel<T, EPI, 1, NCH, 9>), dim3(2 * n_cu), dim3(576), 0, s, p);
      else hipLaunchKernelGGL((gemv_rows_norm_kernel<T, EPI, 1, NCH, F8 == WF_E4M3, 9>), dim3(2 * n_cu), dim3(576), 0, s, p);
      return;
    }
  }
#if OMCHAT_EXPERIMENTS
  if constexpr (EPI == EPI_SWIGLU && RR == 1) {
    const int nwg = cdiv(n_out, 4), xs = (int)(g_gemv_skew < 256u ? g_gemv_skew : 0u);
    if (xs > 0 && nwg % 8 == 0 && n_out % 4 == 0 && xs < nwg / 8) {
      GemvP q = p; q.xskew = xs;
      if constexpr (F8 == WF_MX4) hipLaunchKernelGGL((gemv_rows_norm_mx4_kernel<T, EPI, RR, NCH>), dim3(8 * (nwg / 8 + xs)), dim3(256), 0, s, q);
      else hipLaunchKernelGGL((gemv_rows_norm_kernel<T, EPI, RR, NCH, F8 == WF_E4M3>), dim3(8 * (nwg / 8 + xs)), dim3(256), 0, s, q);
      return;
    }
  }
#endif
  if constexpr (F8 == WF_MX4) hipLaunchKernelGGL((gemv_rows_norm_mx4_kernel<T, EPI, RR, NCH>), dim3(cdiv(cdiv(n_out, RR), 4)), dim3(256), 0, s, p);
  else hipLaunchKernelGGL((gemv_rows_norm_kernel<T, EPI, RR, NCH, F8 == WF_E4M3>), dim3(cdiv(cdiv(n_out, RR), 4)), dim3(256), 0, s, p);
}
template <typename T, int EPI, int RR, int F8>
void launch_rows_norm(const GemvP& p, hipStream_t s) {
  switch (cdiv(p.K, 512)) {
    case 1: launch_rows_norm_n<T, EPI, RR, F8, 1>(p, s); break;
    case 2: launch_rows_norm_n<T, EPI, RR, F8, 2>(p, s); break;
    case 3: launch_rows_norm_n<T, EPI, RR, F8, 3>(p, s); break;
    case 4: launch_rows_norm_n<T, EPI, RR, F8, 4>(p, s); break;
    case 5: launch_rows_norm_n<T, EPI, RR, F8, 5>(p, s); break;
    case 6: launch_rows_norm_n<T, EPI, RR, F8, 6>(p, s); break;
    case 7: launch_rows_norm_n<T, EPI, RR, F8, 7>(p, s); break;
    default: launch_rows_norm_n<T, EPI, RR, F8, 8>(p, s); break;
  }
}

template <int EPI, int NCH>
void launch_rows_norm_x12_n(const GemvP& p, hipStream_t s) {
  constexpr int RR = EPI == EPI_SWIGLU ? 1 : 4;
  const int n_out = EPI == EPI_SWIGLU ? p.N / 2 : p.N;
  hipLaunchKernelGGL((gemv_rows_norm_x12_kernel<bf16, EPI, RR, NCH>), dim3(cdiv(cdiv(n_out, RR), 4)), dim3(256), 0, s, p);
}
template <int EPI>
void launch_rows_norm_x12(const GemvP& p, hipStream_t s) {
  switch (p.K / 512) {
    case 1: launch_rows_norm_x12_n<EPI, 1>(p, s); break;
    case 2: launch_rows_norm_x12_n<EPI, 2>(p, s); break;
    case 3: launch_rows_norm_x12_n<EPI, 3>(p, s); break;
    case 4: launch_rows_norm_x12_n<EPI, 4>(p, s); break;
    case 5: launch_rows_norm_x12_n<EPI, 5>(p, s); break;
    case 6: launch_rows_norm_x12_n<EPI, 6>(p, s); break;
    case 7: launch_rows_norm_x12_n<EPI, 7>(p, s); break;
    default: launch_rows_norm_x12_n<EPI, 8>(p, s); break;
  }
}

template <typename T, int EPI, int RR, int F8>
void launch_rows_r(const GemvP& p, hipStream_t s) {
  const int n_out = EPI == EPI_SWIGLU ? p.N / 2 : p.N;
  if constexpr (RR == 1 && EPI == EPI_RESID) {
    const int n_cu = device_cus();
    if (g_gemv_rows_balance && p.ksplit == 1 && n_out == 7 * 2 * n_cu) {
      if constexpr (F8 == WF_MX4) hipLaunchKernelGGL((gemv_rows_mx4_kernel<T, EPI, 1, 7>), dim3(2 * n_cu, 1), dim3(448), 0, s, p);
      else hipLaunchKernelGGL((gemv_rows_kernel<T, EPI, 1, 7, F8 == WF_E4M3>), dim3(2 * n_cu, 1), dim3(448), 0, s, p);
      return;
    }
  }
  int grid = cdiv(cdiv(n_out, RR), 4);
  grid = grid > 2048 ? 2048 : grid;
  if constexpr (F8 == WF_MX4) hipLaunchKernelGGL((gemv_rows_mx4_kernel<T, EPI, RR, 4>), dim3(grid, p.ksplit), dim3(256), 0, s, p);
  else hipLaunchKernelGGL((gemv_rows_kernel<T, EPI, RR, 4, F8 == WF_E4M3>), dim3(grid, p.ksplit), dim3(256), 0, s, p);
}
template <typename T, int EPI, int WF>
void launch_rows_q(const GemvP& p, hipStream_t s) {
  if constexpr (EPI == EPI_SWIGLU || EPI == EPI_NONE) {
    if (p.norm_w) {
      if (EPI == EPI_NONE && p.N < 32768) launch_rows_norm<T, EPI, 2, WF>(p, s);
      else if (EPI == EPI_SWIGLU && g_gemv_gu_rr8 == 2) launch_rows_norm<T, EPI, 2, WF>(p, s);
      else if (EPI == EPI_SWIGLU && g_gemv_gu_rr8 == 1) launch_rows_norm<T, EPI, 1, WF>(p, s);
      else launch_rows_norm<T, EPI, 4, WF>(p, s);
      return;
    }
  }
  if ((EPI == EPI_NONE || EPI == EPI_RESID) && p.N < 32768) launch_rows_r<T, EPI, 1, WF>(p, s);
  else if (EPI == EPI_NONE) launch_rows_r<T, EPI, 8, WF>(p, s);
  else launch_rows_r<T, EPI, 4, WF>(p, s);
}
template <typename T, int EPI>
void launch_rows(const GemvP& p, hipStream_t s) {
  if (p.mx_s) { launch_rows_q<T, EPI, WF_MX4>(p, s); return; }
  if (p.w_scale) { launch_rows_q<T, EPI, WF_E4M3>(p, s); return; }
  if constexpr (EPI == EPI_SWIGLU || EPI == EPI_NONE) {
    if (p.norm_w) {
      if (EPI == EPI_NONE && p.N < 32768) launch_rows_norm<T, EPI, 2, WF_16>(p, s);
      else if (EPI == EPI_SWIGLU && g_gemv_gu_rr == 2) launch_rows_norm<T, EPI, 2, WF_16>(p, s);
      else if (EPI == EPI_SWIGLU && g_gemv_gu_rr == 3) launch_rows_norm<T, EPI, 3, WF_16>(p, s);
      else if (EPI == EPI_SWIGLU) launch_rows_norm<T, EPI, 1, WF_16>(p, s);
      else launch_rows_norm<T, EPI, 4, WF_16>(p, s);
      return;
    }
  }
  if ((EPI == EPI_NONE || EPI == EPI_RESID) && p.N < 32768) launch_rows_r<T, EPI, 1, WF_16>(p, s);
  else if (EPI == EPI_SWIGLU && (g_gemv_shard & 4) && p.N / 2 < 16 * device_cus()) launch_rows_r<T, EPI, 1, WF_16>(p, s);
  else launch_rows_r<T, EPI, 4, WF_16>(p, s);
}

template <typename T>
int launch_t(const GemvArgs& a, hipStream_t s) {
  const int ks = a.ksplit > 1 ? a.ksplit : 1;
// ... 46 lines not shown
#endif
      if (a.mx_scale) {
        if (a.epi == EPI_SWIGLU) {
          if (a.b > 16) hipLaunchKernelGGL((gemv_xs_mx4_kernel<T, EPI_SWIGLU, 2, 7>), grid, dim3(512), 0, s, p);
          else hipLaunchKernelGGL((gemv_xs_mx4_kernel<T, EPI_SWIGLU, 1, 7>), grid, dim3(512), 0, s, p);
        } else {
          if (a.b > 16) hipLaunchKernelGGL((gemv_xs_mx4_kernel<T, EPI_NONE, 2, 7>), grid, dim3(512), 0, s, p);
          else hipLaunchKernelGGL((gemv_xs_mx4_kernel<T, EPI_NONE, 1, 7>), grid, dim3(512), 0, s, p);
        }
      } else if (a.epi == EPI_SWIGLU) {
        if (a.b > 16) hipLaunchKernelGGL((gemv_xs_kernel<T, EPI_SWIGLU, 2, 7>), grid, dim3(512), 0, s, p);
        else hipLaunchKernelGGL((gemv_xs_kernel<T, EPI_SWIGLU, 1, 7>), grid, dim3(512), 0, s, p);
      } else {
        if (a.b > 16) hipLaunchKernelGGL((gemv_xs_kernel<T, EPI_NONE, 2, 7>), grid, dim3(512), 0, s, p);
        else hipLaunchKernelGGL((gemv_xs_kernel<T, EPI_NONE, 1, 7>), grid, dim3(512), 0, s, p);
      }
      OM_LAUNCH_CHECK();
      return 0;
    }
    if (a.w_packed && !g_gemv_no_xs && a.epi == EPI_PARTIAL && ks > 1 && (a.K >> 6) % 8 == 0 && a.N % 16 == 0) {
      const int q = (a.K >> 6) / 8;
      int a5 = -1;
      for (int t = 0; t <= ks; ++t) if (5 * t + 2 * (ks - t) == q) a5 = t;
      const int n_cu2 = device_cus();
      int gx = std::max(1, n_cu2 / ks);
      const int tiles = a.N / 16;
      if (tiles < 4 * gx && tiles % 2 == 0 && (long)tiles * ks >= n_cu2 && (long)tiles * ks <= 2L * n_cu2) gx = tiles / 2;
      if (a5 >= 0 && (tiles >= 4 * gx || gx == tiles / 2)) {
        const dim3 grid(gx, ks);
        if (a.mx_scale) {
          if (a.b > 16) hipLaunchKernelGGL((gemv_xs_split_mx4_kernel<T, 2>), grid, dim3(512), 0, s, p, a5);
          else hipLaunchKernelGGL((gemv_xs_split_mx4_kernel<T, 1>), grid, dim3(512), 0, s, p, a5);
        } else if (a.b > 16) hipLaunchKernelGGL((gemv_xs_split_kernel<T, 2>), grid, dim3(512), 0, s, p, a5);
        else hipLaunchKernelGGL((gemv_xs_split_kernel<T, 1>), grid, dim3(512), 0, s, p, a5);
        OM_LAUNCH_CHECK();
        return 0;
      }
    }
    if (a.norm_w) { omchat_set_error("launch_gemv: packed-x RMSNorm form: gate|up shape outside the x-stationary launch (N / 32 >= 4 CUs)"); return 1; }
    if (a.epi == EPI_SWIGLU) OM_PK(2, EPI_SWIGLU, 8, 4);
    else if (a.epi == EPI_PARTIAL) {
      const int cps = cdiv(a.K >> 6, ks);
      if ((g_gemv_shard & 2) && cps <= 8) OM_PK(1, EPI_PARTIAL, 8, 1);
      else if ((g_gemv_shard & 2) && cps <= 32) OM_PK(1, EPI_PARTIAL, 8, 2);
      else if (a.K / ks >= 1536) OM_PK(4, EPI_PARTIAL, 4, 2);
      else OM_PK(2, EPI_PARTIAL, 8, 4);
    }
    else if (a.N >= 32768) OM_PK(4, EPI_NONE, 4, 4);
    else OM_PK(2, EPI_NONE, 8, 4);
#undef OM_PK
    OM_LAUNCH_CHECK();
    return 0;
  }
  if (a.x12_top) {
    const bool ok = std::is_same<T, bf16>::value && a.b == 1 && !a.x_packed && !a.w_packed && ks == 1 && a.K >= 512 && a.K % 512 == 0 &&
                    a.ldw == a.K / 2 * 3 && a.x12_cnt && a.x12_patch && !a.w_scale && !a.mx_scale && !a.force_mfma && !g_gemv_force_mfma;
    const bool norm = ok && a.norm_w && (a.epi == EPI_SWIGLU || a.epi == EPI_NONE) && a.K <= RW_MAXC * 512;
    const bool longk = ok && !a.norm_w && a.epi == EPI_RESID && !a.out_f32 && a.K > RW_MAXC * 512 && a.K <= 32768;
    if (!norm && !longk) {
      omchat_set_error("launch_gemv: bf16x12 weights: bf16, b == 1, K % 512 == 0, and norm_w with EPI_SWIGLU / EPI_NONE (K <= 4096) or EPI_RESID on 4096 < K <= 32768");
      return 1;
    }
    if (longk) { const int rc = launch_rows_longk<T>(p, s); if (rc) return rc; }
    else if (a.epi == EPI_SWIGLU) launch_rows_norm_x12<EPI_SWIGLU>(p, s);
    else launch_rows_norm_x12<EPI_NONE>(p, s);
    OM_LAUNCH_CHECK();
    return 0;
  }
  if (a.b == 1 && !a.x_packed && a.epi == EPI_RESID && ks == 1 && !a.out_f32 && a.K > RW_MAXC * 512 && a.K % 8 == 0 && a.K <= 32768 &&
      ((!a.force_mfma && !g_gemv_force_mfma) || a.mx_scale)) {
    const int rc = launch_rows_longk<T>(p, s);
    if (rc) return rc;
    OM_LAUNCH_CHECK();
    return 0;
  }
  const bool rows_ok = a.b == 1 && cdiv(cdiv(a.K, 512), ks) <= RW_MAXC;
  if (a.norm_w && !(rows_ok && ks == 1 && !a.force_mfma && !g_gemv_force_mfma && (a.epi == EPI_NONE || a.epi == EPI_SWIGLU))) {
    omchat_set_error("launch_gemv: the in-register RMSNorm needs the whole-row batch-1 form without split-K (K <= 4096), epilogue NONE / SWIGLU");
    return 1;
  }
  if ((a.w_scale || a.mx_scale) && !rows_ok) { omchat_set_error("launch_gemv: fp8 / MXFP4 weights need b == 1 and <= 8 chunks of 512 per K slice"); return 1; }
  if (rows_ok && (a.w_scale || a.mx_scale || (!a.force_mfma && !g_gemv_force_mfma))) {
    switch (a.epi) {
      case EPI_PARTIAL: launch_rows<T, EPI_PARTIAL>(p, s); break;
      case EPI_SWIGLU: launch_rows<T, EPI_SWIGLU>(p, s); break;
      case EPI_RESID: launch_rows<T, EPI_RESID>(p, s); break;
      default: launch_rows<T, EPI_NONE>(p, s); break;
    }
    OM_LAUNCH_CHECK();
    return 0;
  }
  if (a.b > 16) {
    if (a.epi == EPI_PARTIAL) hipLaunchKernelGGL((gemv_kernel<T, 1, EPI_PARTIAL, 8, 4, false, 2>), dim3(cdiv(a.N, 16), ks), dim3(512), 0, s, p);
    else if (a.epi == EPI_SWIGLU) hipLaunchKernelGGL((gemv_kernel<T, 2, EPI_SWIGLU, 8, 4, false, 2>), dim3(cdiv(a.N, 32)), dim3(512), 0, s, p);
    else if (a.epi == EPI_RESID) hipLaunchKernelGGL((gemv_kernel<T, 1, EPI_RESID, 8, 4, false, 2>), dim3(cdiv(a.N, 16)), dim3(512), 0, s, p);
    else hipLaunchKernelGGL((gemv_kernel<T, 2, EPI_NONE, 8, 4, false, 2>), dim3(cdiv(a.N, 32)), dim3(512), 0, s, p);
    OM_LAUNCH_CHECK();
    return 0;
  }
  if (a.epi == EPI_PARTIAL) {
    if (a.K / 64 / ks <= 32)
      hipLaunchKernelGGL((gemv_kernel<T, 1, EPI_PARTIAL, 4, 8>), dim3(cdiv(a.N, 16), ks), dim3(256), 0, s, p);
    else
      hipLaunchKernelGGL((gemv_kernel<T, 1, EPI_PARTIAL, 8, 4>), dim3(cdiv(a.N, 16), ks), dim3(512), 0, s, p);
  } else if (a.epi == EPI_SWIGLU) {
    hipLaunchKernelGGL((gemv_kernel<T, 2, EPI_SWIGLU, 8, 4>), dim3(cdiv(a.N, 32)), dim3(512), 0, s, p);
  } else if (a.epi == EPI_RESID) {
    hipLaunchKernelGGL((gemv_kernel<T, 1, EPI_RESID, 8, 4>), dim3(cdiv(a.N, 16)), dim3(512), 0, s, p);
  } else {
    if (a.N >= 16384)
      hipLaunchKernelGGL((gemv_kernel<T, 2, EPI_NONE, 8, 8>), dim3(cdiv(a.N, 32)), dim3(512), 0, s, p);
    else
      hipLaunchKernelGGL((gemv_kernel<T, 1, EPI_NONE, 8, 8>), dim3(cdiv(a.N, 16)), dim3(512), 0, s, p);
  }
  OM_LAUNCH_CHECK();
  return 0;
}

}

void gemv_set_force_mfma(int v) { g_gemv_force_mfma = v; }
int gemv_get_force_mfma() { return g_gemv_force_mfma; }
void gemv_set_no_xs(int v) { g_gemv_no_xs = v; }
void gemv_set_shard_shapes(int v) { g_gemv_shard = v; }
int gemv_get_shard_shapes() { return g_gemv_shard; }
void gemv_set_norm_loop(int v) { g_gemv_norm_loop = v; }
void gemv_set_gu_rr(int v) { if (v >= 16) g_gemv_gu_rr8 = v / 16; else g_gemv_gu_rr = v; }
void gemv_set_dyn(int v) { g_gemv_dyn = v; }
void gemv_set_longk_direct(int v) { g_gemv_longk_direct = v; }
void gemv_set_skew(int v) { g_gemv_skew = (unsigned)v; }
void gemv_set_rows_balance(int v) { g_gemv_rows_balance = v; }
int gemv_x12_default_forms() {
  return ((g_gemv_norm_loop & 1) == 0 && g_gemv_gu_rr == 1 && g_gemv_skew == 0u ? 1 : 0) | (g_gemv_longk_direct == 0 ? 2 : 0) | ((g_gemv_norm_loop & 8) == 0 ? 4 : 0);
}

namespace {
template <typename T>
__global__ __launch_bounds__(256) void quant_fp8_rows_kernel(const T* __restrict__ W, int ldw, int N, int K, unsigned char* __restrict__ W8, int ldq,
                                                             float* __restrict__ scale) {
  const int lane = threadIdx.x & 63, n = blockIdx.x * 4 + (threadIdx.x >> 6);
  if (n >= N) return;
  const T* w = W + (size_t)n * ldw;
  float m = 0.f;
  for (int k = lane * 8; k < K; k += 512) {
    const typename V8<T>::type v = ld8<T>(w + k);
#pragma unroll
    for (int j = 0; j < 8; ++j) m = fmaxf(m, fabsf(tof(v[j])));
  }
#pragma unroll
  for (int o = 32; o > 0; o >>= 1) m = fmaxf(m, __shfl_xor(m, o, 64));
  const float sc = m > 0.f ? m / 448.0f : 1.0f;
  if (lane == 0) scale[n] = sc;
  for (int k = lane * 8; k < K; k += 512) {
    const typename V8<T>::type v = ld8<T>(w + k);
    float f[8];
#pragma unroll
    for (int j = 0; j < 8; ++j) f[j] = tof(v[j]) / sc;
    int lo = 0, hi = 0;
    lo = __builtin_amdgcn_cvt_pk_fp8_f32(f[0], f[1], lo, false);
    lo = __builtin_amdgcn_cvt_pk_fp8_f32(f[2], f[3], lo, true);
    hi = __builtin_amdgcn_cvt_pk_fp8_f32(f[4], f[5], hi, false);
    hi = __builtin_amdgcn_cvt_pk_fp8_f32(f[6], f[7], hi, true);
    rw_u32x2 o2 = {(unsigned)lo, (unsigned)hi};
    *reinterpret_cast<rw_u32x2*>(W8 + (size_t)n * ldq + k) = o2;
  }
}
}

int launch_quant_fp8_rows(int dtype, const void* W, int ldw, int N, int K, void* W8, int ld8, float* scale, hipStream_t s) {
  OM_CHECK(K % 8 == 0 && ldw % 8 == 0 && ld8 % 8 == 0, "K, ldw, ld8 must be multiples of 8");
  if (dtype == OMCHAT_F16) hipLaunchKernelGGL(quant_fp8_rows_kernel<f16>, dim3(cdiv(N, 4)), dim3(256), 0, s, (const f16*)W, ldw, N, K, (unsigned char*)W8, ld8, scale);
  else if (dtype == OMCHAT_BF16) hipLaunchKernelGGL(quant_fp8_rows_kernel<bf16>, dim3(cdiv(N, 4)), dim3(256), 0, s, (const bf16*)W, ldw, N, K, (unsigned char*)W8, ld8, scale);
  else { omchat_set_error("launch_quant_fp8_rows: bad dtype"); return 1; }
  OM_LAUNCH_CHECK();
  return 0;
}

namespace {
template <typename T>
__global__ __launch_bounds__(256) void quant_mxfp4_rows_kernel(const T* __restrict__ W, int ldw, int N, int K, unsigned char* __restrict__ W4, int ld4,
                                                               unsigned char* __restrict__ S) {
  const int lane = threadIdx.x & 63, n = blockIdx.x * 4 + (threadIdx.x >> 6);
  if (n >= N) return;
  const T* w = W + (size_t)n * ldw;
  for (int k = lane * 8; k < K; k += 512) {
    const typename V8<T>::type v = ld8<T>(w + k);
// ... 236 lines not shown
```

### omchat_amd/csrc/kernels.h

```cpp
#pragma once
#ifndef OMCHAT_EXPERIMENTS
#define OMCHAT_EXPERIMENTS 0
#endif
#include "common.h"
#if OMCHAT_EXPERIMENTS
#include <hip/hip_ext.h>
extern int g_launch_any_order;
#undef hipLaunchKernelGGL
#define hipLaunchKernelGGL(kernelName, numBlocks, numThreads, memPerBlock, streamId, ...)                                                      \
  do {                                                                                                                                         \
    if (g_launch_any_order)                                                                                                                    \
      hipExtLaunchKernelGGL((kernelName), dim3(numBlocks), dim3(numThreads), (memPerBlock), (streamId), nullptr, nullptr, hipExtAnyOrderLaunch, \
                            __VA_ARGS__);                                                                                                      \
    else                                                                                                                                       \
      hipLaunchKernelGGLInternal((kernelName), numBlocks, numThreads, memPerBlock, streamId, __VA_ARGS__);                                     \
  } while (0)
#endif

enum {
  EPI_NONE = 0,
  EPI_GELU = 1,
  EPI_LS_RESID = 2,
  EPI_RESID = 3,
  EPI_SWIGLU = 4,
// ... 5 lines not shown
};
struct GemmArgs {
  const void* A; int lda;
  const void* W; int ldw;
  void* C; int ldc;
  int M, N, K;
  const void* bias;
  const void* ls;
  const void* resid;
  int ldr;
  int epi;
  int force_tile;
  void* sk_ws; size_t sk_ws_bytes;
  int stream_k;
  int f8;
  const float* a_scale; const float* w_scale;
  const float* row_scale = nullptr;
  const float* rs_stats = nullptr; int rs_ld = 0, rs_nslots = 0, rs_dim = 0; float rs_eps = 0.f;
  float* stats = nullptr; int stats_ld = 0; int* stats_nslots = nullptr;
  const int* lse_labels = nullptr; float* lse_tgt = nullptr;
};
int launch_gemm(int dtype, const GemmArgs& a, hipStream_t stream);
int launch_stats_finish(const float* stats, int ld, int slot0, int nslots, int ngroups, int rows, int dim, float eps, float* out, hipStream_t s);
int launch_row_sumsq(int dtype, const void* x, int ldx, int rows, int H, float* stats, hipStream_t s);
size_t gemm_sk_ws_bytes();
void gemm_set_skew(int v);
void gemm_set_persist(int v);
void gemm_set_wide_store(int v);
void gemm_set_skip_dead(int v);

struct GemvArgs {
  const void* X; int ldx;
  const void* W; int ldw;
  void* Y; int ldy;
  int b, N, K;
  const void* bias;
  const void* resid; int ldr;
  int epi;
  int out_f32;
  int ksplit;
  int force_mfma;
  const float* w_scale;
  int x_packed;
  int w_packed;
  int y_packed;
  const void* norm_w; float norm_eps;
  void* dyn_ctr = nullptr;
  void* y_pack = nullptr;
  unsigned long long* dbg = nullptr;
  const unsigned char* mx_scale = nullptr;
  const unsigned char* x12_top = nullptr;
  const unsigned char* x12_cnt = nullptr;
  const unsigned* x12_patch = nullptr;
};
int launch_encode_bf16x12(const void* W, int ldw, int N, int K, void* coded, unsigned char* top, unsigned char* cnt, unsigned* patch, int* over,
                          hipStream_t stream);
int launch_pack_x(int dtype, const void* X, int ldx, int b, int K, void* out, hipStream_t s);
int launch_pack_w(int dtype, const void* W, int ldw, int N, int K, void* out, hipStream_t s);
int launch_pack_w4(const void* W4, const unsigned char* S, int N, int K, void* W4P, unsigned char* SP, hipStream_t s);
int launch_gemv(int dtype, const GemvArgs& a, hipStream_t stream);
int launch_gemv_wait(int dtype, const GemvArgs& a, const unsigned* flags, unsigned epoch, int nflags, unsigned* err, int mode, hipStream_t s);
int launch_quant_fp8_rows(int dtype, const void* W, int ldw, int N, int K, void* W8, int ld8, float* scale, hipStream_t stream);
int launch_quant_mxfp4_rows(int dtype, const void* W, int ldw, int N, int K, void* W4, int ld4, unsigned char* S, hipStream_t stream);
void gemv_set_force_mfma(int v);
int gemv_get_force_mfma();
void gemm_set_autotune(int v);
int gemm_tune_load(const char* path);
int gemm_tune_dump(const char* path);
long gemm_tune_runs();
void model_set_ar_min_rows(int v);
void model_set_tp_f32(int v);
void model_set_pack_replica(int v);
void model_set_norm_in_gemv(int v);
void model_set_vit_fused(int v);
void model_set_tp_sp(int v);
int launch_fold_cols(int dtype, const void* W, const void* n, void* out, int rows, int cols, hipStream_t s);

int launch_layernorm(int dtype, const void* x, int ldx, const void* w, const void* b, void* y, int ldy, int rows, int H, float eps, hipStream_t stream);
int launch_rmsnorm(int dtype, const void* x, int ldx, const void* w, void* y, int ldy, int rows, int H, float eps, hipStream_t s, int pack_nb = 0);
int launch_rmsnorm_q8(int dtype, const void* x, int ldx, const void* w, void* y8, int ldy, float* scale, int rows, int H, float eps, hipStream_t s);
int launch_quant_rows_q8(int dtype, const void* x, int ldx, void* y8, int ldy, float* scale, int rows, int H, hipStream_t s);
int launch_resid_rmsnorm(int dtype, void* x, int ldx, const float* part, int ks, const void* w, void* xn, int ldn, int rows, int H, float eps,
                         hipStream_t s, int pack_nb = 0);
int launch_resid16_norm(int dtype, void* x, int ldx, const void* y, int ldy, const void* w, const void* b, void* xn, int ldn, int rows, int H, float eps,
                        hipStream_t s);
int launch_vit_qknorm(int dtype, void* qkv, int ld, const void* wq, const void* wk, int rows, int C, int C_total,
                      float eps, float q_scale, const float* sumsq_in, hipStream_t s, int only_k = 0);
int launch_vit_qk_sumsq(int dtype, const void* qkv, int ld, int rows, int C, float* sumsq_out, hipStream_t s);
int launch_vit_knorm_slots(int dtype, void* k, int ld, const void* wk, int rows, int C, int C_total, float eps, const float* stats, int stats_ld, int nslots,
                           float* sumsq_q, hipStream_t s);
struct AttnArgs {
  const void* Q; int64_t q_sb, q_sh, q_sr;
  const void* K; int64_t k_sb, k_sh, k_sr;
  const void* V; int64_t v_sb, v_sh, v_sr;
  void* O; int64_t o_sb, o_sh, o_sr;
  int batch, q_heads, kv_heads;
  int Sq, Skv;
  const int* kv_len;
  const int* kv_start;
  int causal;
  int q_pos0;
  float scale;
  int head_dim;
  const float* qn_sumsq = nullptr; int qn_stride = 0, qn_dim = 0; const void* qn_w = nullptr; float qn_eps = 0.f, qn_scale = 1.f;
};
int launch_attn_prefill(int dtype, const AttnArgs& a, hipStream_t s);
int launch_attn_uniform_rows(int dtype, const AttnArgs& a, hipStream_t s);
void attn_set_v2(int v);
void model_set_fuse_peer_norm(int v);
void attn_set_tpw(int v);
void attn_set_klds(int v);
void attn_set_dma(int v);
void attn_set_dma_slots(int v);
void attn_set_dma_rot(int v);
void attn_set_hsplit(int v);
void attn_set_mha_xcd(int v);
void attn_set_kg(int v);
void attn_set_peel(int v);
void attn_set_kv8_tpw(int v);
void attn_set_kv8_fuse(int v);
void model_set_extend_attn(int v);
void model_set_x12_roles(int v);
void model_set_suffix_attn(int v);
int gemv_x12_default_forms();
bool attn_decode_kv8_fuses_rope(int batch, int kv_heads, int L, bool masked);
void attn_set_merge_mid_min(int v);
void attn_set_merge_dg(int v);
void gemv_set_norm_loop(int v);
void gemv_set_dyn(int v);
void gemv_set_skew(int v);
void gemv_set_rows_balance(int v);
void gemv_set_no_xs(int v);
void gemv_set_shard_shapes(int v);
void gemv_set_gu_rr(int v);
void gemv_set_longk_direct(int v);
void norm_set_wave(int v);
void model_set_ao_oproj(int v);
int gemv_get_shard_shapes();

struct AttnOperands {
  const void* Q; int64_t q_sb, q_sh;
  const void* K; int64_t k_sb, k_sh, k_sr;
  const void* V; int64_t v_sb, v_sh, v_sr;
  void* O; int64_t o_sb, o_sh;
  int q_heads, kv_heads;
  float scale;
  float* ws; size_t ws_bytes;
  const float* rope; int rope_max;
  const void* k_new; const void* v_new; int64_t new_sb;
  int o_pack_nb;
};

struct AttnDecodeArgs : AttnOperands {
  int batch;
  int L;
  const int* kv_len;
  const int* pos;
  const float* k_scale; const float* v_scale; int64_t scale_sb, scale_sh;
  void* k16_w = nullptr; void* v16_w = nullptr;
  const unsigned char* key_mask; int64_t mask_sb;
  unsigned* done_flags = nullptr; unsigned done_epoch = 0; int done_mode = 0;
  unsigned long long* done_dbg = nullptr;
};
int launch_kv_quant(int dtype, const void* kc, const void* vc, void* k8, void* v8, float* ks, float* vs, int b, int kv_heads, int64_t c_sb, int64_t c_sh,
                    int64_t s_sb, int64_t s_sh, const int* pos_lo, int pos0, const int* len, int max_rows, hipStream_t s);
size_t attn_decode_ws_bytes(int batch, int q_heads, int max_len);
int launch_attn_decode(int dtype, const AttnDecodeArgs& a, hipStream_t s);

enum AttnBlockMode { ATTN_VERIFY = 0, ATTN_EXTEND, ATTN_SHARED, ATTN_SUFFIX };
struct AttnBlockArgs : AttnOperands {
  int mode;
  int G, N, S, P, L;
  const int* kv_len;
};
constexpr int VERIFY_MAX_T = 16;
size_t attn_block_ws_bytes(const AttnBlockArgs& a);
// ... 191 lines not shown
```

### omchat_amd/csrc/model.hip

```cpp
#include "ctx.h"
#include <limits.h>
#include <math.h>
#include <string.h>
#include <algorithm>
#include <functional>
#include <string>
#include <unordered_map>
#include <vector>

static thread_local std::string g_err;
void omchat_set_error(const std::string& s) { g_err = s; }
extern "C" const char* omchat_last_error(void) { return g_err.c_str(); }
extern "C" const char* omchat_version(void) { return "omchat_hip 0.1 (gfx950)"; }

namespace {

__global__ void cast_from_f32_f16(const float* s, f16* d, int64_t n) {
  for (int64_t i = (int64_t)blockIdx.x * blockDim.x + threadIdx.x; i < n; i += (int64_t)gridDim.x * blockDim.x) d[i] = (f16)s[i];
}
__global__ void cast_from_f32_bf16(const float* s, bf16* d, int64_t n) {
  for (int64_t i = (int64_t)blockIdx.x * blockDim.x + threadIdx.x; i < n; i += (int64_t)gridDim.x * blockDim.x) d[i] = (bf16)s[i];
}
__global__ void add_positions_kernel(int* pos, int b, int d) {
  const int i = threadIdx.x;
// ... 834 lines not shown
    const int R = std::min(32, n - r0);
    GemvArgs g{(const char*)hidden + (size_t)r0 * H * 2, H, nullptr, 0, logits + (size_t)r0 * V, V, R, V, H, nullptr, nullptr, 0, EPI_NONE, 1};
    use_weight(g, lm);
    g.x_packed = x_packed;
    TRY(launch_gemv(ctx->dt, g, s));
  }
  return 0;
}

static int build_replica(omchat_ctx* ctx, int fmt) {
  omchat_ctx::WTable& T = ctx->wt[fmt];
  if (T.state == omchat_ctx::W_BUILT) return 0;
  const bool f8 = fmt == OMCHAT_WFMT_E4M3, mx = fmt == OMCHAT_WFMT_MXFP4, mxp = fmt == OMCHAT_WFMT_MXFP4_PACKED, p16 = fmt == OMCHAT_WFMT_16_PACKED;
  if (f8 || mx) OM_CHECK(omchat_weights_missing(ctx) == 0, "load the weights before quantising them");
  if (mx) OM_CHECK(ctx->c.t_hidden % 32 == 0 && ctx->t_qdim % 32 == 0 && ctx->c.t_mlp % 32 == 0,
                   "MXFP4 decode: every streamed K (hidden_size, heads x 128, intermediate_size) must be a multiple of 32");
  if (mxp) TRY(build_replica(ctx, OMCHAT_WFMT_MXFP4));
  const std::vector<omchat_ctx::WRef>& src = ctx->wt[mxp ? OMCHAT_WFMT_MXFP4 : OMCHAT_WFMT_16].e;
  if (T.e.empty()) {
    std::vector<omchat_ctx::WRef> fresh(src.size());
    std::vector<void**> slots;
    std::vector<size_t> sizes;
    for (size_t j = 0; j < fresh.size(); ++j) {
      const size_t N = entry_shape(ctx, j).N, K = entry_shape(ctx, j).K;
      omchat_ctx::WRef& r = fresh[j];
      r.ldw = (int)(mx || mxp ? K / 2 : K);
      r.packed = p16 || mxp;
      slots.push_back(&r.W); sizes.push_back(p16 ? N * K * 2 : f8 ? N * K : N * (K / 2));
      if (f8) { slots.push_back((void**)&r.w_scale); sizes.push_back(N * 4); }
      if (mx || mxp) { slots.push_back((void**)&r.mx_scale); sizes.push_back(N * (K / 32)); }
    }
    if (ctx->alloc_group(slots, sizes)) {
      if (p16) { T.state = omchat_ctx::W_UNAVAILABLE; return 0; }
      if (mxp) omchat_set_error("omchat_enable_mxfp4_decode: the packed MXFP4 replica of mode 2 does not fit in device memory (hipMalloc failed)");
      return 2;
    }
    T.e.swap(fresh);
  }
  for (size_t j = 0; j < T.e.size(); ++j) {
    const int N = entry_shape(ctx, j).N, K = entry_shape(ctx, j).K;
    const omchat_ctx::WRef& w = src[j]; const omchat_ctx::WRef& r = T.e[j];
    if (f8) TRY(launch_quant_fp8_rows(ctx->dt, w.W, K, N, K, r.W, K, r.w_scale, nullptr));
    else if (mx) TRY(launch_quant_mxfp4_rows(ctx->dt, w.W, K, N, K, r.W, K / 2, r.mx_scale, nullptr));
    else if (mxp) TRY(launch_pack_w4(w.W, w.mx_scale, N, K, r.W, r.mx_scale, nullptr));
    else TRY(launch_pack_w(ctx->dt, w.W, K, N, K, r.W, nullptr));
  }
  OM_HIP(hipDeviceSynchronize());
  T.state = omchat_ctx::W_BUILT;
  return 0;
}

int g_x12_roles = 7;
void model_set_x12_roles(int v) { g_x12_roles = v & 7; }

static int x12_step_mask(const omchat_ctx* ctx, int rows, int fmt) {
  if (rows != 1 || fmt != OMCHAT_WFMT_16 || ctx->dt != OMCHAT_BF16 || ctx->tp_size != 1) return 0;
  return g_x12_roles & gemv_x12_default_forms();
}

static int build_x12(omchat_ctx* ctx, int role) {
  omchat_ctx::X12Table& T = ctx->x12[role];
  if (T.state == omchat_ctx::W_BUILT || T.state == omchat_ctx::W_UNAVAILABLE) return 0;
  const omchat_config& c = ctx->c;
  const int H = c.t_hidden, It = c.t_mlp, L = c.t_layers;
  const bool lm = role == omchat_ctx::X12_LM, down = role == omchat_ctx::X12_DOWN;
  const size_t N = lm ? c.t_vocab : down ? H : 2 * (size_t)It, K = down ? It : H, n = lm ? 1 : L;
  const bool k_ok = K % 512 == 0 && (down ? (K > 4096 && K <= 32768) : K <= 4096);
  if (!k_ok || omchat_weights_missing(ctx) != 0) { if (!k_ok) T.state = omchat_ctx::W_UNAVAILABLE; return 0; }
  if (T.e.empty()) {
    std::vector<omchat_ctx::X12Ref> fresh(n);
    std::vector<void**> slots;
    std::vector<size_t> sizes;
    for (auto& r : fresh) {
      slots.push_back(&r.W); sizes.push_back(N * (K / 2 * 3));
      slots.push_back((void**)&r.top); sizes.push_back(N);
      slots.push_back((void**)&r.cnt); sizes.push_back(N);
      slots.push_back((void**)&r.patch); sizes.push_back(N * 32 * 4);
    }
    int* over = nullptr;
    if (!ctx->x12_over) { slots.push_back((void**)&over); sizes.push_back((size_t)std::max(L, 1) * 4); }
    if (ctx->alloc_group(slots, sizes)) { T.state = omchat_ctx::W_UNAVAILABLE; return 0; }
    if (over) ctx->x12_over = over;
    T.e.swap(fresh);
  }
  OM_HIP(hipDeviceSynchronize());
  OM_HIP(hipMemset(ctx->x12_over, 0, n * 4));
  for (size_t j = 0; j < n; ++j) {
    const void* W = lm ? ctx->lm_w(OMCHAT_WFMT_16).W : ctx->layer_w(OMCHAT_WFMT_16, (int)j)[down ? omchat_ctx::P_DOWN : omchat_ctx::P_GU].W;
    const omchat_ctx::X12Ref& r = T.e[j];
    TRY(launch_encode_bf16x12(W, (int)K, (int)N, (int)K, r.W, r.top, r.cnt, r.patch, ctx->x12_over + j, nullptr));
  }
  OM_HIP(hipDeviceSynchronize());
  std::vector<int> over(n);
  OM_HIP(hipMemcpy(over.data(), ctx->x12_over, n * 4, hipMemcpyDeviceToHost));
  bool moved = false;
  for (size_t j = 0; j < n; ++j) { moved = moved || (T.state == omchat_ctx::W_STALE && T.e[j].ok != !over[j]); T.e[j].ok = !over[j]; }
  if (moved) drop_decode_graphs(ctx);
  T.state = omchat_ctx::W_BUILT;
  return 0;
}

extern "C" int omchat_enable_fp8_decode(omchat_ctx* ctx, int on) {
  OM_CHECK(ctx, "null context");
  OM_CHECK(ctx->c.t_layers > 0, "context has no decoder");
  if (!on) { ctx->fp8_decode = false; return 0; }
  OM_CHECK(!ctx->mxfp4_mode, "MXFP4 decode is on: one weight format per step (omchat_enable_mxfp4_decode(ctx, 0) first)");
  TRY(build_replica(ctx, OMCHAT_WFMT_E4M3));
  ctx->fp8_decode = true;
  return 0;
}

extern "C" int omchat_enable_mxfp4_decode(omchat_ctx* ctx, int mode) {
  OM_CHECK(ctx, "null context");
  OM_CHECK(ctx->c.t_layers > 0, "context has no decoder");
  OM_CHECK(mode >= 0 && mode <= 2, "mode: 0 = off, 1 = batch-1 steps, 2 = steps of up to 32 rows as well");
  if (!mode) { ctx->mxfp4_mode = 0; return 0; }
  OM_CHECK(!ctx->fp8_decode, "fp8 decode is on: one weight format per step (omchat_enable_fp8_decode(ctx, 0) first)");
  OM_CHECK(ctx->tp_size == 1, "MXFP4 decode under tensor parallelism is not implemented");
  if (mode == 2) {
    const omchat_config& c = ctx->c;
    OM_CHECK(c.t_hidden % 64 == 0 && ctx->t_qdim % 64 == 0 && c.t_mlp % 64 == 0,
             "MXFP4 decode mode 2: the packed path needs hidden_size, heads x 128 and intermediate_size each a multiple of 64");
    OM_CHECK(ctx->t_qkvdim % 16 == 0 && c.t_hidden % 16 == 0 && c.t_vocab % 16 == 0,
             "MXFP4 decode mode 2: the packed path needs the qkv width, hidden_size and vocab_size each a multiple of 16");
  }
  TRY(build_replica(ctx, mode == 2 ? OMCHAT_WFMT_MXFP4_PACKED : OMCHAT_WFMT_MXFP4));
  ctx->mxfp4_mode = mode;
  return 0;
}

extern "C" int omchat_enable_fp8_kv(omchat_ctx* ctx, int on) {
  OM_CHECK(ctx, "null context");
  const omchat_config& c = ctx->c;
  OM_CHECK(c.t_layers > 0, "context has no decoder");
  ctx->kv8_valid = false;
  if (!on) { ctx->fp8_kv = false; return 0; }
  if (!ctx->k8cache) {
    const size_t bytes = (size_t)c.t_layers * ctx->cache_layer_stride();
    const size_t sc = (size_t)c.t_layers * ctx->scale_layer_stride() * 4;
    TRY(ctx->alloc(&ctx->k8cache, bytes)); TRY(ctx->alloc(&ctx->v8cache, bytes));
    TRY(ctx->alloc((void**)&ctx->ks8, sc)); TRY(ctx->alloc((void**)&ctx->vs8, sc));
// ... 331 lines not shown
    return 0;
  };
  auto gemv_partial = [&](const void* X, int ldx, const WRef& W, int K, int ks) -> int {
    OM_CHECK(b <= 32, "split-K decode path handles b <= 32");
    const GemvArgs g = gemv_args(X, ldx, W, K, ctx->tw_part, H, b, H, nullptr, nullptr, EPI_PARTIAL, ks, false);
    TRY(launch_gemv(ctx->dt, g, s));
    return 0;
  };
  const bool fused = b <= 32;
  auto ks_rows = [&](int K) { const int nch = cdiv(K, 512); return nch >= 16 ? std::min(DEC_KS_MAX, nch) : std::max(1, std::min(3, nch)); };
  auto ks_short = [&](int K) { return std::max(1, std::min(DEC_KS_MAX, (K / 64) / 16)); };
  const bool shard_ks = (gemv_get_shard_shapes() & 2) != 0;
  const int ks_o = b == 1 ? ks_rows(qd) : ((wpk || mpk) && qd == 3584 ? 2 : (shard_ks && qd / 64 <= 64) ? ks_short(qd) :
                                           std::max(1, std::min(DEC_KS_MAX, std::min(qd / 64, cdiv(512, cdiv(H, 16))))));
  const int ks_d = b == 1 ? ks_rows(It) : (shard_ks && It / 64 <= 64) ? ks_short(It) :
                                          std::max(1, std::min(DEC_KS_MAX, std::min(It / 64, 3 * cdiv(512, cdiv(H, 16)))));
  const bool tp1_like = ctx->tp_size == 1 || (OMCHAT_EXPERIMENTS && g_shard_as_tp1 && ctx->hook == omchat_allreduce_noop);
  const bool n2 = (g_norm_in_gemv & 1) && fused && b == 1 && tp1_like && qd <= 4096 && H <= 4096 && !gemv_get_force_mfma();
  const bool n1 = n2 && (g_norm_in_gemv & 2) && It <= 32768 && It % 8 == 0;
  const bool nb2 = OMCHAT_EXPERIMENTS && (g_norm_in_gemv & 4) && fused && wpk && ctx->tp_size == 1 && !wq && (qd >> 6) == 56 && (H >> 6) == 56 && qd % 64 == 0 &&
                   H / 16 <= device_cus() && (2 * It) / 32 >= 4 * device_cus();
  const int x12m = n1 ? x12_step_mask(ctx, b, fmt) : 0;
  auto x12_of = [&](int role, size_t j) -> const omchat_ctx::X12Ref* {
    const omchat_ctx::X12Table& T = ctx->x12[role];
    return ((x12m >> role) & 1) && T.state == omchat_ctx::W_BUILT && T.e[j].ok ? &T.e[j] : nullptr;
  };
  if (fused && !n1) TRY(launch_rmsnorm(ctx->dt, x, H, ctx->dl[0].ln1, ctx->tw_xn, H, b, H, c.t_eps, s, pk));
#if OMCHAT_EXPERIMENTS
  if ((g_ao_oproj & 16) && ctx->dbg_stamps) OM_HIP(hipMemsetAsync(ctx->dbg_stamps, 0, (size_t)c.t_layers * 256, s));
#endif
  for (int i = 0; i < c.t_layers; ++i) {
    auto& L = ctx->dl[i];
    const WRef* W = ctx->layer_w(fmt, i);
    const WRef* W16 = ctx->layer_w(OMCHAT_WFMT_16, i);
    char* kc = (char*)ctx->kcache + (size_t)i * ctx->cache_layer_stride() * 2;
    char* vc = (char*)ctx->vcache + (size_t)i * ctx->cache_layer_stride() * 2;
    if (!fused) TRY(launch_rmsnorm(ctx->dt, x, H, L.ln1, ctx->tw_xn, H, b, H, c.t_eps, s));
    if (g_decode_layer && n1 && exact_len && !masked && !wq && !(ctx->fp8_kv && ctx->kv8_valid) && ctx->dl_ws) {
      DecodeLayerArgs d{L.ln1, L.ln2, W16[QKV].W, L.bqkv, W16[O].W, W16[GU].W, W16[DOWN].W, kc, vc, ctx->cache_sh(), x, H, qd, ctx->t_kvdim, It, c.t_heads, c.t_kv_heads, Lmax,
                        ctx->rope, c.max_seq, c.t_eps, omchat_ctx::T_ATTN_SCALE, ctx->dl_ws, ++ctx->fd_epoch, ctx->fd_err, 2000};
      if (decode_layer_ok(d)) {
        const bool mark_l = allow_prof && i == c.t_layers / 2;
        if (mark_l) ctx->prof_mark(OMCHAT_PROF_DECODE_GATEUP, s);
        TRY(launch_decode_layer(ctx->dt, d, s));
        if (mark_l) ctx->prof_mark(OMCHAT_PROF_DECODE_GATEUP, s);
        ++ctx->n_layer_launches;
        continue;
      }
      --ctx->fd_epoch;
    }
    if (n1) {
      GemvArgs g = gemv_args(x, H, W[QKV], H, ctx->tw_qkv, qkvd, 1, qkvd, L.bqkv, nullptr, EPI_NONE, 0, false);
      g.norm_w = L.ln1; g.norm_eps = c.t_eps;
      if (OMCHAT_EXPERIMENTS && (g_ao_oproj & 16) && ctx->dbg_stamps) g.dbg = ctx->dbg_stamps + (size_t)i * 32;
      TRY(launch_gemv(ctx->dt, g, s));
    } else {
      TRY(gemv(ctx->tw_xn, H, W[QKV], H, ctx->tw_qkv, qkvd, qkvd, L.bqkv, nullptr, EPI_NONE));
    }
    AttnDecodeArgs a{};
    ctx->bind_attn(a, i, true);
    a.ws = ctx->tw_attn_ws; a.ws_bytes = ctx->tw_attn_ws_bytes;
    a.o_pack_nb = fused ? pk : 0;
    a.batch = b; a.L = Lmax; a.kv_len = exact_len ? nullptr : ctx->d_len; a.pos = ctx->d_pos;
    if (masked) { a.key_mask = ctx->d_mask; a.mask_sb = ctx->mask_sb; }
    if (ctx->fp8_kv && ctx->kv8_valid) {
      const size_t off = (size_t)i * ctx->cache_layer_stride(), so = (size_t)i * ctx->scale_layer_stride();
      RopeArgs r{ctx->tw_qkv, qkvd, b, 1, c.t_heads, c.t_kv_heads, ctx->d_pos, 0, ctx->rope, c.max_seq, kc, vc, ctx->cache_sb(), ctx->cache_sh()};
      r.k8 = (char*)ctx->k8cache + off; r.v8 = (char*)ctx->v8cache + off; r.ks = ctx->ks8 + so; r.vs = ctx->vs8 + so;
      r.s_sb = (int64_t)c.t_kv_heads * c.max_seq; r.s_sh = c.max_seq;
      if (masked) r.slot0 = Lmax - 1;
      else if (exact_len) { r.pos = nullptr; r.pos0 = Lmax - 1; }
      if (attn_decode_kv8_fuses_rope(b, c.t_kv_heads, Lmax, masked)) { a.k16_w = kc; a.v16_w = vc; a.pos = nullptr; }
      else {
        TRY(launch_rope_kv(ctx->dt, r, s));
        a.rope = nullptr; a.pos = nullptr; a.k_new = nullptr; a.v_new = nullptr;
      }
      a.K = (char*)ctx->k8cache + off; a.V = (char*)ctx->v8cache + off;
      a.k_scale = ctx->ks8 + so; a.v_scale = ctx->vs8 + so; a.scale_sb = (int64_t)c.t_kv_heads * c.max_seq; a.scale_sh = c.max_seq;
    }
    bool ao_oproj = false;
    const bool fuse_ao = g_fuse_attn_oproj && n2 && exact_len && !wq && a.rope && ctx->fd_ws && attn_oproj_fused_ok(a, H, qd);
    if (vL < 0 && ctx->group.on()) {
      const GroupState& G = ctx->group;
      AttnBlockArgs sa{};
      static_cast<AttnOperands&>(sa) = a;
      sa.ws = (float*)G.ws.p; sa.ws_bytes = G.ws.cap;
      sa.mode = ATTN_SHARED; sa.G = G.b; sa.N = G.N; sa.P = G.P; sa.L = Lmax; sa.kv_len = ctx->d_len;
      TRY(launch_attn_block(ctx->dt, sa, s));
    } else if (vL >= 0) {
      AttnBlockArgs va{};
      static_cast<AttnOperands&>(va) = a;
      va.mode = ATTN_VERIFY; va.S = b; va.L = vL;
      TRY(launch_attn_block(ctx->dt, va, s));
    } else if (fuse_ao) {
      FusedDecodeArgs fa{W16[O].W, qd, x, H, qd, ctx->fd_ws, ++ctx->fd_epoch, ctx->fd_err, 2000};
      TRY(launch_attn_oproj_fused(ctx->dt, a, fa, s));
      ++ctx->n_fused_launches;
    } else {
#if OMCHAT_EXPERIMENTS
      ao_oproj = (g_ao_oproj & 1) && n2 && !wq && !masked && ctx->fd_ws && Lmax <= 4096 && H == 3584 && qd == 3584 && c.t_heads <= 64 && !ctx->graph_on;
      if (ao_oproj) { a.done_flags = (unsigned*)ctx->fd_ws; a.done_epoch = ++ctx->fd_epoch; a.done_mode = g_ao_oproj; }
      if ((g_ao_oproj & 16) && n2 && ctx->dbg_stamps) a.done_dbg = ctx->dbg_stamps + (size_t)i * 32;
#endif
      TRY(launch_attn_decode(ctx->dt, a, s));
    }
    if (fuse_ao) {
    } else if (ao_oproj) {
      GemvArgs g = gemv_args(ctx->tw_ao, qd, W16[O], qd, x, H, 1, H, nullptr, x, EPI_RESID, 0, false);
      if ((g_ao_oproj & 16) && ctx->dbg_stamps) g.dbg = ctx->dbg_stamps + (size_t)i * 32;
      TRY(launch_gemv_wait(ctx->dt, g, (const unsigned*)ctx->fd_ws, ctx->fd_epoch, c.t_heads, ctx->fd_err, g_ao_oproj, s));
    } else if (n2 && OMCHAT_EXPERIMENTS && (g_ao_oproj & 16) && ctx->dbg_stamps && !wq) {
      GemvArgs g = gemv_args(ctx->tw_ao, qd, W16[O], qd, x, H, 1, H, nullptr, x, EPI_RESID, 0, false);
      g.dbg = ctx->dbg_stamps + (size_t)i * 32;
      TRY(launch_gemv(ctx->dt, g, s));
    } else if (n2) {
      TRY(gemv(ctx->tw_ao, qd, W[O], qd, x, H, H, nullptr, x, EPI_RESID));
    } else if (nb2) {
      GemvArgs g = gemv_args(ctx->tw_ao, qd, W[O], qd, x, H, b, H, nullptr, x, EPI_RESID, 0, false);
      g.y_pack = ctx->tw_xn;
      TRY(launch_gemv(ctx->dt, g, s));
    } else if (fused) {
      TRY(gemv_partial(ctx->tw_ao, qd, W[O], qd, ks_o));
      TRY(ctx->reduce_resid_rmsnorm(x, H, ctx->tw_part, ks_o, L.ln2, ctx->tw_xn, H, b, H, c.t_eps, pk, s));
    } else if (ctx->tp_size == 1) {
      TRY(gemv(ctx->tw_ao, qd, W[O], qd, x, H, H, nullptr, x, EPI_RESID));
    } else {
      TRY(gemv(ctx->tw_ao, qd, W[O], qd, y, H, H, nullptr, lead ? x : nullptr, lead ? EPI_RESID : EPI_NONE));
      TRY(ctx->allreduce(y, (size_t)b * H, s));
      std::swap(x, y);
    }
    if (!fused) TRY(launch_rmsnorm(ctx->dt, x, H, L.ln2, ctx->tw_xn, H, b, H, c.t_eps, s));
    const bool mark = allow_prof && i == c.t_layers / 2;
    if (mark) ctx->prof_mark(OMCHAT_PROF_DECODE_GATEUP, s);
    if (n2) {
      GemvArgs g = gemv_args(x, H, W[GU], H, ctx->tw_act, It, 1, 2 * It, nullptr, nullptr, EPI_SWIGLU, 0, false);
      g.norm_w = L.ln2; g.norm_eps = c.t_eps;
      if (const auto* r = x12_of(omchat_ctx::X12_GU, i)) { use_weight_x12(g, *r, H); ++ctx->x12_launches[omchat_ctx::X12_GU]; }
      if (ctx->dyn_ctr && !ctx->graph_on) g.dyn_ctr = ctx->dyn_ctr + (size_t)i * 65 * 64;
      if (OMCHAT_EXPERIMENTS && (g_ao_oproj & 16) && ctx->dbg_stamps) g.dbg = ctx->dbg_stamps + (size_t)i * 32;
      TRY(launch_gemv(ctx->dt, g, s));
    } else if (nb2) {
      GemvArgs g = gemv_args(ctx->tw_xn, H, W[GU], H, ctx->tw_act, It, b, 2 * It, nullptr, nullptr, EPI_SWIGLU, 0, true);
      g.norm_w = L.ln2; g.norm_eps = c.t_eps;
      TRY(launch_gemv(ctx->dt, g, s));
    } else {
      TRY(gemv(ctx->tw_xn, H, W[GU], H, ctx->tw_act, It, 2 * It, nullptr, nullptr, EPI_SWIGLU, true));
    }
    if (mark) ctx->prof_mark(OMCHAT_PROF_DECODE_GATEUP, s);
    if (n1 && OMCHAT_EXPERIMENTS && (g_ao_oproj & 16) && ctx->dbg_stamps && !wq) {
      GemvArgs g = gemv_args(ctx->tw_act, It, W16[DOWN], It, x, H, 1, H, nullptr, x, EPI_RESID, 0, false);
      g.dbg = ctx->dbg_stamps + (size_t)i * 32;
      TRY(launch_gemv(ctx->dt, g, s));
    } else if (n1 && x12_of(omchat_ctx::X12_DOWN, i)) {
      GemvArgs g = gemv_args(ctx->tw_act, It, W[DOWN], It, x, H, 1, H, nullptr, x, EPI_RESID, 0, false);
      use_weight_x12(g, *x12_of(omchat_ctx::X12_DOWN, i), It);
      ++ctx->x12_launches[omchat_ctx::X12_DOWN];
      TRY(launch_gemv(ctx->dt, g, s));
    } else if (n1) {
      TRY(gemv(ctx->tw_act, It, W[DOWN], It, x, H, H, nullptr, x, EPI_RESID));
    } else if (fused) {
      TRY(gemv_partial(ctx->tw_act, It, W[DOWN], It, ks_d));
      const void* nw = i + 1 < c.t_layers ? ctx->dl[i + 1].ln1 : ctx->t_norm;
      TRY(ctx->reduce_resid_rmsnorm(x, H, ctx->tw_part, ks_d, nw, ctx->tw_xn, H, b, H, c.t_eps, pk, s));
    } else if (ctx->tp_size == 1) {
      TRY(gemv(ctx->tw_act, It, W[DOWN], It, x, H, H, nullptr, x, EPI_RESID));
    } else {
      TRY(gemv(ctx->tw_act, It, W[DOWN], It, y, H, H, nullptr, lead ? x : nullptr, lead ? EPI_RESID : EPI_NONE));
// ... 1 lines not shown
      std::swap(x, y);
    }
  }
  if (!fused)   TRY(launch_rmsnorm(ctx->dt, x, H, ctx->t_norm, ctx->tw_xn, H, b, H, c.t_eps, s));
  float* lg = logits ? logits : ctx->tw_logits;
  if (n1) {
    GemvArgs g{x, H, nullptr, 0, lg, c.t_vocab, 1, c.t_vocab, H, nullptr, nullptr, 0, EPI_NONE, 1};
    use_weight(g, ctx->lm_w(fmt));
    if (const auto* r = x12_of(omchat_ctx::X12_LM, 0)) { use_weight_x12(g, *r, H); ++ctx->x12_launches[omchat_ctx::X12_LM]; }
    g.norm_w = ctx->t_norm; g.norm_eps = c.t_eps;
    TRY(launch_gemv(ctx->dt, g, s));
  } else {
    TRY(lm_head_rows(ctx, ctx->tw_xn, b, lg, s, ctx->lm_w(fmt), fused && pk));
  }
  if (vL >= 0) TRY(pick_verify(ctx, lg, b, tokens, next_tokens, s, vsample));
  else if (next_tokens) TRY(pick_run(ctx, lg, b, next_tokens, s, true, tokens));
  else {
    hipLaunchKernelGGL(advance_lens_kernel, dim3(1), dim3(64 > b ? 64 : b), 0, s, ctx->d_pos, ctx->d_len, b);
    TRY(pick_feed(ctx, tokens, b, s));
  }
  OM_LAUNCH_CHECK();
  return 0;
}

static void destroy_graph(omchat_ctx::DecodeGraph& g) {
  if (g.exec) (void)hipGraphExecDestroy(g.exec);
  if (g.graph) (void)hipGraphDestroy(g.graph);
  g = omchat_ctx::DecodeGraph{};
}

void drop_decode_graphs(omchat_ctx* ctx) {
  for (auto& kv : ctx->graphs) destroy_graph(kv.second);
  ctx->graphs.clear();
}


extern "C" int omchat_enable_decode_graph(omchat_ctx* ctx, int on) {
  OM_CHECK(ctx, "null ctx");
  OM_CHECK(ctx->c.t_layers > 0, "context has no decoder");
  if (on && !ctx->graph_stream) {
    OM_HIP(hipStreamCreateWithFlags(&ctx->graph_stream, hipStreamNonBlocking));
    OM_HIP(hipEventCreateWithFlags(&ctx->graph_ev_in, hipEventDisableTiming));
    OM_HIP(hipEventCreateWithFlags(&ctx->graph_ev_out, hipEventDisableTiming));
    TRY(ctx->alloc((void**)&ctx->d_tok_in, (size_t)ctx->c.max_batch * 4));
    TRY(ctx->alloc((void**)&ctx->d_tok_out, (size_t)ctx->c.max_batch * 4));
  }
  ctx->graph_on = on != 0;
  return 0;
}

extern "C" int omchat_bf16x12_stats(omchat_ctx* ctx, int* roles, long* launches, int* coded) {
  OM_CHECK(ctx, "null context");
  if (roles) *roles = g_x12_roles;
  for (int r = 0; r < omchat_ctx::X12_ROLES; ++r) {
    if (launches) launches[r] = ctx->x12_launches[r];
    int n = 0;
    if (ctx->x12[r].state == omchat_ctx::W_BUILT) for (const auto& e : ctx->x12[r].e) n += e.ok ? 1 : 0;
    if (coded) coded[r] = n;
  }
  return 0;
}

extern "C" int omchat_decode_graph_stats(omchat_ctx* ctx, long* steps, long* replays, long* captures) {
  OM_CHECK(ctx, "null ctx");
  if (steps) *steps = ctx->graph_steps;
  if (replays) *replays = ctx->graph_replays;
  if (captures) *captures = ctx->graph_captures;
  return 0;
}

extern "C" int omchat_decode_step(omchat_ctx* ctx, const int32_t* tokens, int b, float* logits, int32_t* next_tokens, void* stream) {
  OM_CHECK(ctx && tokens, "null argument");
  const omchat_config& c = ctx->c;
  OM_CHECK(c.t_layers > 0, "context has no decoder");
  OM_CHECK(b >= 1 && b <= c.max_batch, "batch exceeds max_batch");
  OM_CHECK(mx4_rows_ok(ctx, b), MX4_ROWS_MSG);
  int Lmax = 0;
  OM_CHECK(!ctx->left_padded, "per-sequence decode after a left-padded prefill: use omchat_decode_step_masked (the reference positions such a "
                              "batch with sum(mask) - 1 and a per-row key mask, omchat_arch.py:61-70; DESIGN.md section 7)");
  OM_CHECK(ctx->dec_mode != 2, "omchat_decode_step after omchat_decode_step_masked on the same prefill: the two place the cache rows differently");
  bool same_len = true;
  int Lmin = c.max_seq;
  for (int i = 0; i < b; ++i) {
    OM_CHECK(ctx->h_len[i] >= 1, "decode before prefill");
    Lmax = std::max(Lmax, ctx->h_len[i] + 1);
    Lmin = std::min(Lmin, ctx->h_len[i]);
    same_len = same_len && ctx->h_len[i] == ctx->h_len[0];
  }
  OM_CHECK(Lmax <= c.max_seq, "KV cache full (max_seq)");
  hipStream_t s = (hipStream_t)stream;
  GroupState& G = ctx->group;
  const bool grp = G.on();
  if (grp) {
    OM_CHECK(b == G.b * G.N && Lmin >= G.P, "a sampled group shares its prompt: a step takes all its b * N rows, none shorter than the prompt (omchat_group_begin with b = 0 first)");
    OM_CHECK(ctx->tp_size == 1 && !(ctx->fp8_kv && ctx->kv8_valid), "shared-prompt mode: one GPU, 16-bit KV cache");
    Lmax = std::min(c.max_seq, G.P + (Lmax - G.P + 255) / 256 * 256);
    const size_t need = attn_shared_ws_bytes(G.b, G.N, c.t_heads, c.t_kv_heads, G.P, Lmax);
    if (need > G.ws.cap) TRY(ctx->grow(G.ws, attn_shared_ws_bytes(G.b, G.N, c.t_heads, c.t_kv_heads, G.P, std::min(c.max_seq, Lmax + 768))));
  }
  TRY(step_weights_ready(ctx, b));
  TRY(pick_admit(ctx, next_tokens != nullptr, true));
  ctx->graph_steps++;
  const bool graph = ctx->graph_on && ctx->tp_size == 1 && b <= 32 && !(ctx->prof_on && ctx->graph_steps % 8 == 0);
  if (!graph) {
    TRY(decode_body(ctx, tokens, b, Lmax, logits, next_tokens, s, true, same_len && !grp));
  } else {
    const int fmt = step_format(ctx, b);
    omchat_ctx::DecodeGraph& g = ctx->graphs[b * 8 + (is_mxfp4(fmt) ? 4 : 0) + (fmt == OMCHAT_WFMT_E4M3 ? 2 : 0) + ((ctx->fp8_kv && ctx->kv8_valid) ? 1 : 0) +
                                             (grp ? (1 << 20) : 0) + (x12_step_mask(ctx, b, fmt) << 21)];
    hipStream_t gs = ctx->graph_stream;
    OM_HIP(hipEventRecord(ctx->graph_ev_in, s));
// ... 302 lines not shown
```

### omchat_amd/engine.py

```python
import ctypes as C
import numpy as np

from . import _lib
from ._lib import OmchatConfig, check, ptr, cur_stream
from .config import OmChatConfig


def _torch():
    import torch
    return torch


GROUP_SHARE_P_MIN = 2048


def group_share_refusal(fp8_kv, tp_size, q_heads, kv_heads, N):
    if fp8_kv:
        return "the e4m3 KV cache"
    if tp_size != 1:
        return "tensor parallelism"
    if not 2 <= N <= 16 or N * (q_heads // max(1, kv_heads)) > 128:
        return "N outside 2 <= N <= 16 and N * (q heads per kv head) <= 128"
    return None

# ... 109 lines not shown
            check(self.lib.omchat_ctx_allreduce(self.h, ptr(t), t.numel(), _lib.dtype_code(t.dtype), cur_stream()))
        return t

    def encode_images_dp(self, tower, pixels, select_layer=-1):
        torch = _torch()
        n = pixels.shape[0]
        out = torch.zeros(n, self.ntok, self.cfg.text["hidden_size"], dtype=self.torch_dtype, device=self.device)
        lo, hi = self.tp_rank * n // self.tp_size, (self.tp_rank + 1) * n // self.tp_size
        if hi > lo:
            out[lo:hi] = tower.encode_images(pixels[lo:hi], select_layer)
        return self.allreduce(out)

    def comm_stats(self):
        a, b = C.c_long(0), C.c_long(0)
        check(self.lib.omchat_ctx_comm_stats(self.h, C.byref(a), C.byref(b)))
        rs, ag = C.c_long(0), C.c_long(0)
        check(self.lib.omchat_ctx_sp_stats(self.h, C.byref(rs), C.byref(ag)))
        return dict(peer_allreduces=a.value, rccl_allreduces=b.value, sp_reduce_scatters=rs.value, sp_all_gathers=ag.value)

    def enable_fp8_decode(self, on=True):
        check(self.lib.omchat_enable_fp8_decode(self.h, int(on)))

    def enable_mxfp4_decode(self, on=True, batched=False):
        check(self.lib.omchat_enable_mxfp4_decode(self.h, (2 if batched else 1) if on else 0))
        self._mxfp4_decode = bool(on)
        self._mxfp4_batched = bool(on) and bool(batched)

    def enable_fp8_kv(self, on=True):
        check(self.lib.omchat_enable_fp8_kv(self.h, int(on)))
        self._fp8_kv = bool(on)
        self._prefix = None

    def masked_decode_supported(self):
        return self.tp_size == 1

    def enable_fp8_prefill(self, on=True):
        check(self.lib.omchat_enable_fp8_prefill(self.h, int(on)))
        self._fp8_prefill = bool(on)
        self._prefix = None

    def enable_decode_graph(self, on=True):
        check(self.lib.omchat_enable_decode_graph(self.h, int(on)))

    def decode_graph_stats(self):
        st, rp, cp = C.c_long(0), C.c_long(0), C.c_long(0)
        check(self.lib.omchat_decode_graph_stats(self.h, C.byref(st), C.byref(rp), C.byref(cp)))
        return dict(steps=st.value, replays=rp.value, captures=cp.value)

    def bf16x12_stats(self):
        roles, launches, coded = C.c_int(0), (C.c_long * 3)(), (C.c_int * 3)()
        check(self.lib.omchat_bf16x12_stats(self.h, C.byref(roles), launches, coded))
        return dict(roles=roles.value, launches=list(launches), coded=list(coded))

    def prof_enable(self, on=True):
        check(self.lib.omchat_prof_enable(self.h, int(on)))

    def prof_read(self, cat, reset=True):
        ms, n = C.c_double(0), C.c_long(0)
        check(self.lib.omchat_prof_read(self.h, cat, C.byref(ms), C.byref(n), int(reset)))
        return ms.value, n.value

    def device_bytes(self):
        return int(self.lib.omchat_device_bytes(self.h))

    def _px(self, pixels):
        torch = _torch()
        if pixels.dim() != 4 or pixels.shape[1] != 3:
            raise ValueError(f"wrong pixel_values size: {tuple(pixels.shape)}")
        s = self.cfg.vision["image_size"]
        if pixels.shape[2] != s or pixels.shape[3] != s:
            raise ValueError(f"expected {s}x{s} tiles, got {tuple(pixels.shape[2:])}")
        return pixels.to(device=self.device, dtype=self.torch_dtype).contiguous()

    def vit_forward(self, pixels, select_layer=-1, select_feature="patch"):
        torch = _torch()
        if select_feature not in ("patch", "cls_patch"):
            raise ValueError(f"Unexpected select feature: {select_feature}")
        px = self._px(pixels)
        n = px.shape[0]
        keep = select_feature == "cls_patch"
        out = torch.empty(n, self.ntok + (1 if keep else 0), self.cfg.vision["hidden_size"], dtype=self.torch_dtype, device=self.device)
        check(self.lib.omchat_vit_forward(self.h, ptr(px), n, select_layer, int(keep), ptr(out), cur_stream()))
        return out

    def projector_forward(self, x):
        torch = _torch()
        x = x.to(device=self.device, dtype=self.torch_dtype).contiguous()
        rows = x.numel() // x.shape[-1]
        out = torch.empty(*x.shape[:-1], self.cfg.text["hidden_size"], dtype=self.torch_dtype, device=self.device)
        check(self.lib.omchat_projector_forward(self.h, ptr(x), rows, ptr(out), cur_stream()))
        return out

    def encode_images(self, pixels, select_layer=-1):
        torch = _torch()
        px = self._px(pixels)
        n = px.shape[0]
        out = torch.empty(n, self.ntok, self.cfg.text["hidden_size"], dtype=self.torch_dtype, device=self.device)
        check(self.lib.omchat_encode_images(self.h, ptr(px), n, select_layer, ptr(out), cur_stream()))
        self._enc_st["calls"] += 1; self._enc_st["tiles"] += n
        return out

    def encode_stats(self, reset=False):
        out = dict(self._enc_st)
        if reset:
            self._enc_st = dict(calls=0, tiles=0)
        return out
# ... 414 lines not shown
```

Before: 383.1.

## Extend bf16x12 compressed weights to QKV and O projections in decode

Adds short-K bf16x12 GEMV kernels for the fused-norm QKV projection and the residual O projection, plus encoding of those weights at build time. By default only the O-projection role is on (short roles = 2). The aim is to cut weight bytes read per decode step for attention projections at TP=1. The cost is extra device memory for the coded tables, a decode step on the patch/escape path, and new kernel variants with their own scheduling.

```diff
diff --git a/include/omchat_hip.h b/include/omchat_hip.h
--- a/include/omchat_hip.h
+++ b/include/omchat_hip.h
@@ -129,6 +129,7 @@
 int omchat_enable_decode_graph(omchat_ctx* ctx, int on);
 int omchat_decode_graph_stats(omchat_ctx* ctx, long* steps, long* replays, long* captures);
 int omchat_bf16x12_stats(omchat_ctx* ctx, int* roles, long* launches, int* coded);
+int omchat_bf16x12_short_stats(omchat_ctx* ctx, int* roles, long* launches, int* coded);
 
 int omchat_enable_fp8_decode(omchat_ctx* ctx, int on);
 
@@ -204,6 +205,9 @@
 int omchat_op_encode_bf16x12(const void* W, int N, int K, void* coded, void* top, void* cnt, void* patch, void* over, void* stream);
 int omchat_op_gemv_bf16x12(const void* X, const void* coded, const void* top, const void* cnt, const void* patch, void* Y, int N, int K,
                            const void* norm_w, float eps, const void* resid, int epi, int out_f32, void* stream);
+int omchat_op_gemv_bf16x12_short(int dtype, const void* X, const void* coded, const void* top, const void* cnt, const void* patch, void* Y,
+                                 int b, int N, int K, const void* bias, const void* norm_w, float eps, const void* resid, int epi, int out_f32,
+                                 void* stream);
 int omchat_op_pack_w(int dtype, const void* W, int ldw, int N, int K, void* out, void* stream);
 int omchat_op_pack_w4(const void* W4, const void* S, int N, int K, void* W4P, void* SP, void* stream);
 int omchat_op_gemv_prepacked(int dtype, const void* XP, const void* WP, const void* SP, void* Y, int ldy, int b, int N, int K, const void* bias,
diff --git a/omchat_amd/_lib.py b/omchat_amd/_lib.py
--- a/omchat_amd/_lib.py
+++ b/omchat_amd/_lib.py
@@ -119,6 +119,8 @@
     "omchat_op_gemv_prepacked": (_i, [_i, _vp, _vp, _vp, _vp, _i, _i, _i, _i, _vp, _i, _i, _i, _i, _vp]),
     "omchat_op_encode_bf16x12": (_i, [_vp, _i, _i, _vp, _vp, _vp, _vp, _vp, _vp]),
     "omchat_op_gemv_bf16x12": (_i, [_vp, _vp, _vp, _vp, _vp, _vp, _i, _i, _vp, _f, _vp, _i, _i, _vp]),
+    "omchat_op_gemv_bf16x12_short": (_i, [_i, _vp, _vp, _vp, _vp, _vp, _vp, _i, _i, _i, _vp, _vp, _f, _vp, _i, _i, _vp]),
+    "omchat_bf16x12_short_stats": (_i, [_vp, C.POINTER(_i), C.POINTER(C.c_long), C.POINTER(_i)]),
     "omchat_op_gemv_mxfp4_norm": (_i, [_i, _vp, _vp, _vp, _vp, _i, _i, _vp, _f, _vp, _i, _i, _vp]),
     "omchat_op_rmsnorm": (_i, [_i, _vp, _vp, _vp, _i, _i, _f, _vp]),
     "omchat_op_resid_rmsnorm": (_i, [_i, _vp, _i, _vp, _i, _vp, _vp, _i, _i, _i, _f, _i, _vp]),
diff --git a/omchat_amd/csrc/capi.hip b/omchat_amd/csrc/capi.hip
--- a/omchat_amd/csrc/capi.hip
+++ b/omchat_amd/csrc/capi.hip
@@ -96,6 +96,7 @@
   if (key == 48) { attn_set_kv8_fuse(value); return 0; }
   if (key == 49) { model_set_extend_attn(value); return 0; }
   if (key == 50) { model_set_x12_roles(value); return 0; }
+  if (key == 52) { model_set_x12_short_roles(value); return 0; }
   if (key == 51) { model_set_suffix_attn(value); return 0; }
   if (key == 38) { gemv_set_gu_rr(value); return 0; }
   if (key == 39) { gemv_set_longk_direct(value); return 0; }
@@ -900,6 +901,16 @@
   g.x12_top = (const unsigned char*)top; g.x12_cnt = (const unsigned char*)cnt; g.x12_patch = (const unsigned*)patch;
   return launch_gemv(OMCHAT_BF16, g, S(stream));
 }
+extern "C" int omchat_op_gemv_bf16x12_short(int dtype, const void* X, const void* coded, const void* top, const void* cnt, const void* patch, void* Y,
+                                            int b, int N, int K, const void* bias, const void* norm_w, float eps, const void* resid, int epi, int out_f32,
+                                            void* stream) {
+  OM_CHECK(X && coded && top && cnt && patch && Y, "null argument");
+  GemvArgs g{X, K, coded, K / 2 * 3, Y, N, b, N, K, bias, resid, N, epi, out_f32};
+  g.norm_w = norm_w; g.norm_eps = eps;
+  g.x12_top = (const unsigned char*)top; g.x12_cnt = (const unsigned char*)cnt; g.x12_patch = (const unsigned*)patch;
+  g.x12_short = 1;
+  return launch_gemv(dtype, g, S(stream));
+}
 
 extern "C" int omchat_op_attn_prefill_d(int dtype, const void* q, const void* k, const void* v, void* out, int b, int Sq, int Skv, int Hq,
                                         int Hkv, int D, const int32_t* kv_len, int causal, int q_pos0, float scale, void* stream) {
diff --git a/omchat_amd/csrc/ctx.h b/omchat_amd/csrc/ctx.h
--- a/omchat_amd/csrc/ctx.h
+++ b/omchat_amd/csrc/ctx.h
@@ -130,12 +130,12 @@
   const WRef* layer_w(int fmt, int layer) const { return &wt[fmt].e[(size_t)layer * 4]; }
   const WRef& lm_w(int fmt) const { return wt[fmt].e.back(); }
   bool built(int fmt) const { return wt[fmt].state == W_BUILT; }
-  enum X12Role { X12_GU = 0, X12_DOWN = 1, X12_LM = 2, X12_ROLES = 3 };
+  enum X12Role { X12_GU = 0, X12_DOWN = 1, X12_LM = 2, X12_LONG_ROLES = 3, X12_QKV = 3, X12_O = 4, X12_ROLES = 5 };
   struct X12Ref { void* W = nullptr; unsigned char* top = nullptr; unsigned char* cnt = nullptr; unsigned* patch = nullptr; bool ok = false; };
   struct X12Table { std::vector<X12Ref> e; int state = W_ABSENT; };
   X12Table x12[X12_ROLES];
   int* x12_over = nullptr;
-  long x12_launches[X12_ROLES] = {0, 0, 0};
+  long x12_launches[X12_ROLES] = {0, 0, 0, 0, 0};
   bool fp8_decode = false;
   int mxfp4_mode = 0;
   void *k8cache = nullptr, *v8cache = nullptr;
diff --git a/omchat_amd/csrc/gemv.hip b/omchat_amd/csrc/gemv.hip
--- a/omchat_amd/csrc/gemv.hip
+++ b/omchat_amd/csrc/gemv.hip
@@ -729,6 +729,19 @@
   }
 }
 
+constexpr int X12_SHORT_G = 2;
+template <typename T, int C0, int GS, int NCH>
+__device__ __forceinline__ void x12_dot_groups(const X12W* w, X12Row& s, const rw_u32x4* xr, int lane, float& a) {
+  if constexpr (C0 < NCH) {
+    constexpr int G = NCH - C0 < GS ? NCH - C0 : GS;
+    rw_u32x4 wd[G];
+    x12_group<G>(wd, w + C0, s, C0, NCH, lane);
+#pragma unroll
+    for (int c = 0; c < G; ++c) a = rw_dot8<T>(wd[c], xr[C0 + c], a);
+    x12_dot_groups<T, C0 + GS, GS, NCH>(w, s, xr, lane, a);
+  }
+}
+
 template <typename T, int WF>
 __device__ __forceinline__ typename RwW<WF>::type rw_ldw(const GemvP& p, size_t row, int k) {
   if constexpr (WF == WF_X12) return x12_ldw(p, row, k >> 9, (k >> 3) & 63); else
@@ -824,6 +837,41 @@
   }
 }
 
+template <typename T, int R, int NCH>
+__device__ __forceinline__ void rw_rows_x12(const GemvP& p, const int (&rows)[R], int lane, const rw_u32x4 (&xr)[RW_MAXC], float (&acc)[R],
+                                            RwTail<T, R>& tail) {
+  X12W w[R][NCH];
+  X12Row xst[R];
+#pragma unroll
+  for (int r = 0; r < R; ++r)
+#pragma unroll
+    for (int c = 0; c < NCH; ++c) {
+      w[r][c] = x12_ldw(p, (size_t)rows[r], c, lane);
+      if (c == 0) x12_row_load(xst[r], p, (size_t)rows[r], lane);
+      __builtin_amdgcn_sched_barrier(0);
+    }
+  rw_tail_load<T, R>(tail);
+  __builtin_amdgcn_sched_barrier(0);
+#pragma unroll
+  for (int r = 0; r < R; ++r) {
+    x12_row_finish(xst[r]);
+    float a = 0.f;
+    x12_dot_groups<T, 0, X12_SHORT_G, NCH>(&w[r][0], xst[r], &xr[0], lane, a);
+#pragma unroll
+    for (int o = 32; o > 0; o >>= 1) a += __shfl_xor(a, o, 64);
+    acc[r] = a;
+  }
+}
+
+template <typename T, int R, int N>
+__device__ __forceinline__ void rw_dispatch_x12(int nch, const GemvP& p, const int (&rows)[R], int lane, const rw_u32x4 (&xr)[RW_MAXC],
+                                                float (&acc)[R], RwTail<T, R>& tail) {
+  if constexpr (N > 0) {
+    if (nch == N) rw_rows_x12<T, R, N>(p, rows, lane, xr, acc, tail);
+    else rw_dispatch_x12<T, R, N - 1>(nch, p, rows, lane, xr, acc, tail);
+  }
+}
+
 template <typename T, int EPI, int RR, int WAVES, int F8>
 __device__ __forceinline__ void gemv_rows_body(const GemvP& p) {
   constexpr int R = EPI == EPI_SWIGLU ? 2 * RR : RR;
@@ -870,7 +918,8 @@
       if (!hb) tail.p0 = tail.p1;
       if (!hr) tail.p1 = tail.p0;
     }
-    if constexpr (F8 != WF_16) rw_dispatch_q<T, R, RW_MAXC, F8>(nch, p, rows, k0, lane, xr, acc, tail);
+    if constexpr (F8 == WF_X12) rw_dispatch_x12<T, R, RW_MAXC>(nch, p, rows, lane, xr, acc, tail);
+    else if constexpr (F8 != WF_16) rw_dispatch_q<T, R, RW_MAXC, F8>(nch, p, rows, k0, lane, xr, acc, tail);
     else rw_dispatch<T, R, RW_MAXC>(nch, W, p.ldw, rows, k0, p.K, lane, xr, acc, tail);
     if (lane == 0) {
 #pragma unroll
@@ -901,8 +950,10 @@
 __global__ __launch_bounds__(WAVES * 64) void gemv_rows_kernel(GemvP p) { gemv_rows_body<T, EPI, RR, WAVES, F8 ? WF_E4M3 : WF_16>(p); }
 template <typename T, int EPI, int RR, int WAVES>
 __global__ __launch_bounds__(WAVES * 64) void gemv_rows_mx4_kernel(GemvP p) { gemv_rows_body<T, EPI, RR, WAVES, WF_MX4>(p); }
-
-template <typename T, int EPI, int RR, int NCH, int F8, int WAVES>
+template <typename T, int WAVES>
+__global__ __launch_bounds__(WAVES * 64) void gemv_oproj_x12_kernel(GemvP p) { gemv_rows_body<T, EPI_RESID, 1, WAVES, WF_X12>(p); }
+
+template <typename T, int EPI, int RR, int NCH, int F8, int WAVES, bool X12_EARLY = false>
 __device__ __forceinline__ void gemv_rows_norm_body(const GemvP& p) {
   typedef typename V8<T>::type v8;
   constexpr int R = EPI == EPI_SWIGLU ? 2 * RR : RR;
@@ -959,6 +1010,8 @@
   }
   typedef typename RwW<F8>::type wreg_t;
   wreg_t w[R][NCH];
+  constexpr bool XE = X12_EARLY && F8 == WF_X12;
+  X12Row xst[F8 == WF_X12 ? R : 1];
 #pragma unroll
   for (int r = 0; r < R; ++r)
 #pragma unroll
@@ -967,6 +1020,7 @@
       k = k < p.K ? k : 0;
       if constexpr (F8 == WF_X12) w[r][c] = x12_ldw(p, (size_t)rows[r], c, lane);
       else w[r][c] = rw_ldw<T, F8>(p, (size_t)rows[r], k);
+      if constexpr (XE) { if (c == 0) x12_row_load(xst[r], p, (size_t)rows[r], lane); __builtin_amdgcn_sched_barrier(0); }
     }
   float e_bias[RR], e_scale[R];
   {
@@ -988,8 +1042,7 @@
       for (int r = 0; r < R; ++r) e_scale[r] = p.w_scale[rows[r]];
     }
   }
-  X12Row xst[F8 == WF_X12 ? R : 1];
-  if constexpr (F8 == WF_X12) {
+  if constexpr (F8 == WF_X12 && !XE) {
 #pragma unroll
     for (int r = 0; r < R; ++r) x12_row_load(xst[r], p, (size_t)rows[r], lane);
   }
@@ -1036,7 +1089,8 @@
     for (int c = 0; c < NCH; ++c) {
       if constexpr (F8 != WF_X12) a = rw_dotw<T, F8>(w[r][c], xr[c], a);
     }
-    if constexpr (F8 == WF_X12) {
+    if constexpr (XE) x12_dot_groups<T, 0, X12_SHORT_G, NCH>(&w[r][0], xst[r], &xr[0], lane, a);
+    else if constexpr (F8 == WF_X12) {
       constexpr int G0 = NCH < 4 ? NCH : 4, G1 = NCH - G0;
       {
         rw_u32x4 wd[G0];
@@ -1081,6 +1135,8 @@
 __global__ __launch_bounds__(WAVES * 64) void gemv_rows_norm_mx4_kernel(GemvP p) { gemv_rows_norm_body<T, EPI, RR, NCH, WF_MX4, WAVES>(p); }
 template <typename T, int EPI, int RR, int NCH>
 __global__ __launch_bounds__(256) void gemv_rows_norm_x12_kernel(GemvP p) { gemv_rows_norm_body<T, EPI, RR, NCH, WF_X12, 4>(p); }
+template <typename T, int RR, int NCH, int WAVES>
+__global__ __launch_bounds__(WAVES * 64) void gemv_qkv_x12_kernel(GemvP p) { gemv_rows_norm_body<T, EPI_NONE, RR, NCH, WF_X12, WAVES, true>(p); }
 
 template <typename T, int EPI, int NCH, int F8>
 __device__ __forceinline__ void gemv_rows_norm_loop_body(const GemvP& p, int per_wg, unsigned skew) {
@@ -1649,6 +1705,40 @@
   }
 }
 
+template <int NCH>
+void launch_qkv_x12_n(const GemvP& p, hipStream_t s) {
+  if constexpr (NCH >= 4) {
+    const int n_cu = device_cus();
+    if (g_gemv_rows_balance && p.N == 9 * 2 * n_cu) {
+      hipLaunchKernelGGL((gemv_qkv_x12_kernel<bf16, 1, NCH, 9>), dim3(2 * n_cu), dim3(576), 0, s, p);
+      return;
+    }
+  }
+  hipLaunchKernelGGL((gemv_qkv_x12_kernel<bf16, 2, NCH, 4>), dim3(cdiv(cdiv(p.N, 2), 4)), dim3(256), 0, s, p);
+}
+void launch_qkv_x12(const GemvP& p, hipStream_t s) {
+  switch (p.K / 512) {
+    case 1: launch_qkv_x12_n<1>(p, s); break;
+    case 2: launch_qkv_x12_n<2>(p, s); break;
+    case 3: launch_qkv_x12_n<3>(p, s); break;
+    case 4: launch_qkv_x12_n<4>(p, s); break;
+    case 5: launch_qkv_x12_n<5>(p, s); break;
+    case 6: launch_qkv_x12_n<6>(p, s); break;
+    case 7: launch_qkv_x12_n<7>(p, s); break;
+    default: launch_qkv_x12_n<8>(p, s); break;
+  }
+}
+void launch_oproj_x12(const GemvP& p, hipStream_t s) {
+  const int n_cu = device_cus();
+  if (g_gemv_rows_balance && p.N == 7 * 2 * n_cu) {
+    hipLaunchKernelGGL((gemv_oproj_x12_kernel<bf16, 7>), dim3(2 * n_cu, 1), dim3(448), 0, s, p);
+    return;
+  }
+  int grid = cdiv(p.N, 4);
+  grid = grid > 2048 ? 2048 : grid;
+  hipLaunchKernelGGL((gemv_oproj_x12_kernel<bf16, 4>), dim3(grid, 1), dim3(256), 0, s, p);
+}
+
 template <typename T, int EPI, int RR, int F8>
 void launch_rows_r(const GemvP& p, hipStream_t s) {
   const int n_out = EPI == EPI_SWIGLU ? p.N / 2 : p.N;
@@ -1801,9 +1891,21 @@
     OM_LAUNCH_CHECK();
     return 0;
   }
+  if (a.x12_short && !a.x12_top) { omchat_set_error("launch_gemv: x12_short without bf16x12 operands"); return 1; }
   if (a.x12_top) {
     const bool ok = std::is_same<T, bf16>::value && a.b == 1 && !a.x_packed && !a.w_packed && ks == 1 && a.K >= 512 && a.K % 512 == 0 &&
                     a.ldw == a.K / 2 * 3 && a.x12_cnt && a.x12_patch && !a.w_scale && !a.mx_scale && !a.force_mfma && !g_gemv_force_mfma;
+    if (a.x12_short) {
+      const bool k_ok = ok && a.K <= RW_MAXC * 512 && a.N < 32768;
+      const bool qkv = k_ok && a.norm_w && a.epi == EPI_NONE, o = k_ok && !a.norm_w && a.epi == EPI_RESID && !a.out_f32 && a.resid;
+      if (!qkv && !o) {
+        omchat_set_error("launch_gemv: short bf16x12 rows: bf16, b == 1, no split-K, K % 512 == 0, 512 <= K <= 4096, N < 32768, and norm_w with EPI_NONE or EPI_RESID (16-bit output) without it");
+        return 1;
+      }
+      if constexpr (std::is_same<T, bf16>::value) { if (qkv) launch_qkv_x12(p, s); else launch_oproj_x12(p, s); }
+      OM_LAUNCH_CHECK();
+      return 0;
+    }
     const bool norm = ok && a.norm_w && (a.epi == EPI_SWIGLU || a.epi == EPI_NONE) && a.K <= RW_MAXC * 512;
     const bool longk = ok && !a.norm_w && a.epi == EPI_RESID && !a.out_f32 && a.K > RW_MAXC * 512 && a.K <= 32768;
     if (!norm && !longk) {
@@ -1880,7 +1982,8 @@
 void gemv_set_skew(int v) { g_gemv_skew = (unsigned)v; }
 void gemv_set_rows_balance(int v) { g_gemv_rows_balance = v; }
 int gemv_x12_default_forms() {
-  return ((g_gemv_norm_loop & 1) == 0 && g_gemv_gu_rr == 1 && g_gemv_skew == 0u ? 1 : 0) | (g_gemv_longk_direct == 0 ? 2 : 0) | ((g_gemv_norm_loop & 8) == 0 ? 4 : 0);
+  return ((g_gemv_norm_loop & 1) == 0 && g_gemv_gu_rr == 1 && g_gemv_skew == 0u ? 1 : 0) | (g_gemv_longk_direct == 0 ? 2 : 0) | ((g_gemv_norm_loop & 8) == 0 ? 4 : 0) |
+         ((g_gemv_norm_loop & 2) == 0 ? 8 : 0) | 16;
 }
 
 namespace {
diff --git a/omchat_amd/csrc/kernels.h b/omchat_amd/csrc/kernels.h
--- a/omchat_amd/csrc/kernels.h
+++ b/omchat_amd/csrc/kernels.h
@@ -81,6 +81,7 @@
   const unsigned char* x12_top = nullptr;
   const unsigned char* x12_cnt = nullptr;
   const unsigned* x12_patch = nullptr;
+  int x12_short = 0;
 };
 int launch_encode_bf16x12(const void* W, int ldw, int N, int K, void* coded, unsigned char* top, unsigned char* cnt, unsigned* patch, int* over,
                           hipStream_t stream);
@@ -151,6 +152,7 @@
 void model_set_extend_attn(int v);
 void model_set_x12_roles(int v);
 void model_set_suffix_attn(int v);
+void model_set_x12_short_roles(int v);
 int gemv_x12_default_forms();
 bool attn_decode_kv8_fuses_rope(int batch, int kv_heads, int L, bool masked);
 void attn_set_merge_mid_min(int v);
diff --git a/omchat_amd/csrc/model.hip b/omchat_amd/csrc/model.hip
--- a/omchat_amd/csrc/model.hip
+++ b/omchat_amd/csrc/model.hip
@@ -910,10 +910,12 @@
 
 int g_x12_roles = 7;
 void model_set_x12_roles(int v) { g_x12_roles = v & 7; }
+int g_x12_short_roles = 2;
+void model_set_x12_short_roles(int v) { g_x12_short_roles = v & 3; }
 
 static int x12_step_mask(const omchat_ctx* ctx, int rows, int fmt) {
   if (rows != 1 || fmt != OMCHAT_WFMT_16 || ctx->dt != OMCHAT_BF16 || ctx->tp_size != 1) return 0;
-  return g_x12_roles & gemv_x12_default_forms();
+  return (g_x12_roles | (g_x12_short_roles << omchat_ctx::X12_LONG_ROLES)) & gemv_x12_default_forms();
 }
 
 static int build_x12(omchat_ctx* ctx, int role) {
@@ -921,8 +923,9 @@
   if (T.state == omchat_ctx::W_BUILT || T.state == omchat_ctx::W_UNAVAILABLE) return 0;
   const omchat_config& c = ctx->c;
   const int H = c.t_hidden, It = c.t_mlp, L = c.t_layers;
-  const bool lm = role == omchat_ctx::X12_LM, down = role == omchat_ctx::X12_DOWN;
-  const size_t N = lm ? c.t_vocab : down ? H : 2 * (size_t)It, K = down ? It : H, n = lm ? 1 : L;
+  const bool lm = role == omchat_ctx::X12_LM, down = role == omchat_ctx::X12_DOWN, qkv = role == omchat_ctx::X12_QKV, o = role == omchat_ctx::X12_O;
+  const size_t N = lm ? c.t_vocab : (down || o) ? H : qkv ? ctx->t_qkvdim : 2 * (size_t)It, K = down ? It : o ? ctx->t_qdim : H, n = lm ? 1 : L;
+  const int proj = down ? omchat_ctx::P_DOWN : qkv ? omchat_ctx::P_QKV : o ? omchat_ctx::P_O : omchat_ctx::P_GU;
   const bool k_ok = K % 512 == 0 && (down ? (K > 4096 && K <= 32768) : K <= 4096);
   if (!k_ok || omchat_weights_missing(ctx) != 0) { if (!k_ok) T.state = omchat_ctx::W_UNAVAILABLE; return 0; }
   if (T.e.empty()) {
@@ -944,7 +947,7 @@
   OM_HIP(hipDeviceSynchronize());
   OM_HIP(hipMemset(ctx->x12_over, 0, n * 4));
   for (size_t j = 0; j < n; ++j) {
-    const void* W = lm ? ctx->lm_w(OMCHAT_WFMT_16).W : ctx->layer_w(OMCHAT_WFMT_16, (int)j)[down ? omchat_ctx::P_DOWN : omchat_ctx::P_GU].W;
+    const void* W = lm ? ctx->lm_w(OMCHAT_WFMT_16).W : ctx->layer_w(OMCHAT_WFMT_16, (int)j)[proj].W;
     const omchat_ctx::X12Ref& r = T.e[j];
     TRY(launch_encode_bf16x12(W, (int)K, (int)N, (int)K, r.W, r.top, r.cnt, r.patch, ctx->x12_over + j, nullptr));
   }
@@ -1382,6 +1385,7 @@
     if (n1) {
       GemvArgs g = gemv_args(x, H, W[QKV], H, ctx->tw_qkv, qkvd, 1, qkvd, L.bqkv, nullptr, EPI_NONE, 0, false);
       g.norm_w = L.ln1; g.norm_eps = c.t_eps;
+      if (const auto* r = x12_of(omchat_ctx::X12_QKV, i)) { use_weight_x12(g, *r, H); g.x12_short = 1; ++ctx->x12_launches[omchat_ctx::X12_QKV]; }
       if (OMCHAT_EXPERIMENTS && (g_ao_oproj & 16) && ctx->dbg_stamps) g.dbg = ctx->dbg_stamps + (size_t)i * 32;
       TRY(launch_gemv(ctx->dt, g, s));
     } else {
@@ -1443,6 +1447,12 @@
       GemvArgs g = gemv_args(ctx->tw_ao, qd, W16[O], qd, x, H, 1, H, nullptr, x, EPI_RESID, 0, false);
       g.dbg = ctx->dbg_stamps + (size_t)i * 32;
       TRY(launch_gemv(ctx->dt, g, s));
+    } else if (n2 && x12_of(omchat_ctx::X12_O, i)) {
+      GemvArgs g = gemv_args(ctx->tw_ao, qd, W[O], qd, x, H, 1, H, nullptr, x, EPI_RESID, 0, false);
+      use_weight_x12(g, *x12_of(omchat_ctx::X12_O, i), qd);
+      g.x12_short = 1;
+      ++ctx->x12_launches[omchat_ctx::X12_O];
+      TRY(launch_gemv(ctx->dt, g, s));
     } else if (n2) {
       TRY(gemv(ctx->tw_ao, qd, W[O], qd, x, H, H, nullptr, x, EPI_RESID));
     } else if (nb2) {
@@ -1550,11 +1560,23 @@
 extern "C" int omchat_bf16x12_stats(omchat_ctx* ctx, int* roles, long* launches, int* coded) {
   OM_CHECK(ctx, "null context");
   if (roles) *roles = g_x12_roles;
-  for (int r = 0; r < omchat_ctx::X12_ROLES; ++r) {
+  for (int r = 0; r < omchat_ctx::X12_LONG_ROLES; ++r) {
     if (launches) launches[r] = ctx->x12_launches[r];
     int n = 0;
     if (ctx->x12[r].state == omchat_ctx::W_BUILT) for (const auto& e : ctx->x12[r].e) n += e.ok ? 1 : 0;
     if (coded) coded[r] = n;
+  }
+  return 0;
+}
+extern "C" int omchat_bf16x12_short_stats(omchat_ctx* ctx, int* roles, long* launches, int* coded) {
+  OM_CHECK(ctx, "null context");
+  if (roles) *roles = g_x12_short_roles;
+  for (int r = omchat_ctx::X12_LONG_ROLES; r < omchat_ctx::X12_ROLES; ++r) {
+    const int j = r - omchat_ctx::X12_LONG_ROLES;
+    if (launches) launches[j] = ctx->x12_launches[r];
+    int n = 0;
+    if (ctx->x12[r].state == omchat_ctx::W_BUILT) for (const auto& e : ctx->x12[r].e) n += e.ok ? 1 : 0;
+    if (coded) coded[j] = n;
   }
   return 0;
 }
diff --git a/omchat_amd/engine.py b/omchat_amd/engine.py
--- a/omchat_amd/engine.py
+++ b/omchat_amd/engine.py
@@ -185,6 +185,11 @@
         check(self.lib.omchat_bf16x12_stats(self.h, C.byref(roles), launches, coded))
         return dict(roles=roles.value, launches=list(launches), coded=list(coded))
 
+    def bf16x12_short_stats(self):
+        roles, launches, coded = C.c_int(0), (C.c_long * 2)(), (C.c_int * 2)()
+        check(self.lib.omchat_bf16x12_short_stats(self.h, C.byref(roles), launches, coded))
+        return dict(roles=roles.value, launches=list(launches), coded=list(coded))
+
     def prof_enable(self, on=True):
         check(self.lib.omchat_prof_enable(self.h, int(on)))
 
```

Result: no change. 384.4 (median of 6 runs) (+0.3%).
